# V-Sekai/godot-whisper

Hardware: AMD Instinct MI355X
Metric: realtime-factor (audio-sec/wall-sec), base.en 30 s chunk, PCM->tokens (higher is better)
Workload: dtype f16; 1 GPU; base.en, single 30 s chunk per step per GPU (1x MI355X), greedy decode, host params (max_tokens=16, single_segment, token_timestamps), whisper_full with host PCM (H2D inside the timed region); weights=synthetic seed 1234 (f16 ggml, base.en shape)

## Files before the change

### godot-whisper_amd/csrc/api.cpp

```cpp

#include <algorithm>
#include "wmi.h"
#include "kernels.h"

#include <chrono>
#include <cmath>
#include <cstdarg>
#include <cstring>
#include <mutex>
#include <exception>
#include <fstream>

namespace wmi {

namespace {
void default_log(ggml_log_level, const char * text, void *) { fputs(text, stderr); fflush(stderr); }
ggml_log_callback g_log_cb = default_log;
void * g_log_ud = nullptr;
std::recursive_mutex g_log_mu;
}

void log_msg(ggml_log_level lvl, const char * fmt, ...) {
    va_list ap, ap2;
    va_start(ap, fmt);
// ... 312 lines not shown
        ctx->dsp_scratch = nullptr; ctx->dsp_scratch_bytes = 0;
        if (!HIP_OK(hipMalloc((void **) &ctx->dsp_scratch, bytes))) return nullptr;
        ctx->dsp_scratch_bytes = bytes;
    }
    return ctx->dsp_scratch;
}

int wmi_downmix_stereo(struct whisper_context * ctx, const float * frames, int n_frames, int on_device, float * mono_out) {
    if (!ctx || !ctx->state || ctx->host_only || !frames || !mono_out || n_frames < 0) return -1;
    CtxScope lk(ctx);
    if (!HIP_OK(hipSetDevice(ctx->device))) return -2;
    hipStream_t s = ctx->state->dev.stream;
    if (n_frames == 0) return 0;
    if (on_device) { k::downmix_stereo(frames, n_frames, mono_out, s); return HIP_OK(hipStreamSynchronize(s)) ? 0 : -3; }
    float * d_in = dsp_scratch(ctx, (size_t) n_frames * 12), * d_out = d_in ? d_in + (size_t) n_frames * 2 : nullptr;
    bool ok = d_in && HIP_OK(hipMemcpyAsync(d_in, frames, (size_t) n_frames * 8, hipMemcpyHostToDevice, s));
    if (ok) k::downmix_stereo(d_in, n_frames, d_out, s);
    ok = ok && HIP_OK(hipMemcpyAsync(mono_out, d_out, (size_t) n_frames * 4, hipMemcpyDeviceToHost, s)) && HIP_OK(hipStreamSynchronize(s));
    return ok ? 0 : -3;
}

int wmi_resample(struct whisper_context * ctx, const float * src, int n_frames, int src_rate, int dst_rate, int converter, int on_device,
                 float * dst, int dst_capacity) {
    if (!ctx || !ctx->state || ctx->host_only || !src || !dst || n_frames < 0 || src_rate <= 0 || dst_rate <= 0 || dst_capacity < 0 ||
        converter < 0 || converter > 4) return -1;
    CtxScope lk(ctx);
    if (!HIP_OK(hipSetDevice(ctx->device))) return -2;
    hipStream_t s = ctx->state->dev.stream;
    if (src_rate == dst_rate) {
        if (n_frames > dst_capacity) return -4;
        const bool ok = n_frames == 0 || (HIP_OK(hipMemcpyAsync(dst, src, (size_t) n_frames * 4, on_device ? hipMemcpyDeviceToDevice : hipMemcpyHostToHost, s)) &&
                                          HIP_OK(hipStreamSynchronize(s)));
        return ok ? n_frames : -3;
    }
    const double ratio = (double) (uint32_t) dst_rate / (double) (uint32_t) src_rate;
    const long long out_frames = (int) ((uint32_t) n_frames * ratio);
    if (out_frames > dst_capacity) return -4;
    try {
    const k::ResamplePlan pl = k::resample_plan(n_frames, out_frames, ratio, converter);
    if (pl.error == -31) {
        WMI_ERR("wmi_resample: SRC_LINEAR cannot upsample a single frame, 0 frames\n");
        return 0;
    }
    if (pl.error) {
        WMI_ERR("wmi_resample: converter error %d (src_simple would report it through src_strerror)\n", -pl.error);
        return pl.error == -10 ? -10 : 0;
    }
    if (pl.n_out == 0) return 0;
    const float * d_tab = nullptr;
    bool ok = true;
    if (converter <= 2) {
        float *& d_sinc = ctx->d_sinc[converter];
        if (!d_sinc) {
            const float * coeffs; int count, inc;
            (void) k::sinc_table(converter, &coeffs, &count, &inc);
            ok = HIP_OK(hipMalloc((void **) &d_sinc, (size_t) count * 4)) && HIP_OK(hipMemcpyAsync(d_sinc, coeffs, (size_t) count * 4, hipMemcpyHostToDevice, s));
            if (!ok) { if (d_sinc) { (void) hipFree(d_sinc); d_sinc = nullptr; } return -3; }
        }
        d_tab = d_sinc;
    }
    float * d_in = nullptr, * d_out = nullptr; int * d_pos = nullptr; double * d_frac = nullptr;
    const float * in = src; float * out = dst;
    if (!on_device) {
        d_in = dsp_scratch(ctx, ((size_t) std::max(n_frames, 1) + (size_t) pl.n_out) * 4);
        d_out = d_in ? d_in + std::max(n_frames, 1) : nullptr;
        ok = d_in && HIP_OK(hipMemcpyAsync(d_in, src, (size_t) n_frames * 4, hipMemcpyHostToDevice, s));
        in = d_in; out = d_out;
    }
    if (ok && pl.need_table) {
        const int * hp; const double * hf;
        k::resample_table(pl, &hp, &hf);
        ok = HIP_OK(hipMalloc((void **) &d_pos, (size_t) pl.n_out * 4)) && HIP_OK(hipMalloc((void **) &d_frac, (size_t) pl.n_out * 8)) &&
             HIP_OK(hipMemcpyAsync(d_pos, hp, (size_t) pl.n_out * 4, hipMemcpyHostToDevice, s)) &&
             HIP_OK(hipMemcpyAsync(d_frac, hf, (size_t) pl.n_out * 8, hipMemcpyHostToDevice, s));
    }
    if (ok) k::resample_launch(pl, in, n_frames, out, d_tab, d_pos, d_frac, s);
    if (ok && !on_device) ok = HIP_OK(hipMemcpyAsync(dst, d_out, (size_t) pl.n_out * 4, hipMemcpyDeviceToHost, s));
    ok = ok && HIP_OK(hipStreamSynchronize(s));
    (void) hipFree(d_pos); (void) hipFree(d_frac);
    return ok ? (int) pl.n_out : -3;
    } catch (...) { WMI_ERR("wmi_resample: out of memory\n"); return -3; }
}

int wmi_selftest_ts_refine(struct whisper_context * ctx, const float * envelope, int n, const int * s0s1, int n_tok, float * sums, float * thold, int * walks) {
    if (!ctx || !envelope || n <= 0 || !s0s1 || n_tok <= 0 || n_tok > 4096 || !sums || !thold || !walks) return -1;
    CtxScope lk(ctx);
    if (!compute_ready(*ctx, __func__)) return -2;
    try {
        (void) hipSetDevice(ctx->device);
        const size_t nb = (size_t) n / 256 + 2;
        std::vector<float> ext(2 * nb, 0.0f);
        for (size_t b = 0; b * 256 < (size_t) n; ++b) {
            float lo = INFINITY, hi = -INFINITY;
            for (size_t i = b * 256; i < std::min<size_t>((b + 1) * 256, (size_t) n); ++i) { lo = std::min(lo, envelope[i]); hi = std::max(hi, envelope[i]); }
            ext[b] = lo; ext[nb + b] = hi;
        }
        std::vector<k::TsTok> in(n_tok);
        for (int t = 0; t < n_tok; ++t) {
            const int s0 = s0s1[2 * t], s1 = s0s1[2 * t + 1];
            if (s0 < 0 || s0 >= n || s1 < 0 || s1 >= n) return -1;
            in[t] = k::TsTok{ s0, s1, std::max(s0 - 2000, 0), std::min(s1 + 2000, n), nullptr, 0, 0 };
        }
        float * d_en = nullptr, * d_ext = nullptr; k::TsTok * d_in = nullptr; k::TsOut * d_out = nullptr;
        hipStream_t s = ctx->state->dev.stream;
        bool ok = HIP_OK(hipMalloc((void **) &d_en, (size_t) n * 4)) && HIP_OK(hipMalloc((void **) &d_ext, 2 * nb * 4)) &&
                  HIP_OK(hipMalloc((void **) &d_in, (size_t) n_tok * sizeof(k::TsTok))) && HIP_OK(hipMalloc((void **) &d_out, (size_t) n_tok * sizeof(k::TsOut)));
        std::vector<k::TsOut> out(n_tok);
        if (ok) {
            ok = HIP_OK(hipMemcpyAsync(d_en, envelope, (size_t) n * 4, hipMemcpyHostToDevice, s)) &&
                 HIP_OK(hipMemcpyAsync(d_ext, ext.data(), 2 * nb * 4, hipMemcpyHostToDevice, s)) &&
                 HIP_OK(hipMemcpyAsync(d_in, in.data(), (size_t) n_tok * sizeof(k::TsTok), hipMemcpyHostToDevice, s));
            if (ok) k::ts_refine(d_en, d_ext, d_ext + nb, n, d_in, d_out, n_tok, s);
            ok = ok && HIP_OK(hipMemcpyAsync(out.data(), d_out, (size_t) n_tok * sizeof(k::TsOut), hipMemcpyDeviceToHost, s)) && HIP_OK(hipStreamSynchronize(s));
        }
        if (d_en) (void) hipFree(d_en); if (d_ext) (void) hipFree(d_ext); if (d_in) (void) hipFree(d_in); if (d_out) (void) hipFree(d_out);
        if (!ok) return -3;
        for (int t = 0; t < n_tok; ++t) {
            sums[t] = out[t].sum; thold[t] = out[t].thold;
            int * w = walks + 6 * t;
            w[0] = out[t].e0; w[1] = out[t].e1; w[2] = out[t].w_down_above_s0; w[3] = out[t].w_up_below_s0; w[4] = out[t].w_up_above_s1; w[5] = out[t].w_down_below_s1;
        }
        return 0;
    } catch (const std::exception & e) {
        WMI_ERR("%s: %s\n", __func__, e.what());
        return -9;
    }
}

int wmi_selftest_greedy_step(struct whisper_context * ctx, whisper_token token, int pos, float * logits, whisper_token_data * out, int * forms) {
    if (!ctx || ctx->host_only || !out) return -1;
    CtxScope lk(ctx);
    if (!compute_ready(*ctx, __func__)) return -2;
    (void) hipSetDevice(ctx->device);
    BusyScope busy(ctx->device);
    const Vocab & v = ctx->model.vocab;
    if (pos < 0 || pos >= ctx->model.hp.n_text_ctx || token < 0 || token >= v.n_vocab) return -1;
    if (!upload_static_ban(*ctx, whisper_full_default_params(WHISPER_SAMPLING_GREEDY))) return -3;
    StepFilter f{};
    f.ban_blank = false; f.last_ts = false; f.penult_ts = false; f.ts_floor_end = v.beg; f.ts_initial_start = v.n_vocab;
    unsigned fm = 0;
    if (!decode_greedy_step(*ctx, token, pos, f, *out, &fm)) return -4;
    if (logits) {
        DeviceState & d = ctx->state->dev;
        if (!HIP_OK(hipMemcpyAsync(logits, d.logits, (size_t) ctx->model.hp.n_vocab * 4, hipMemcpyDeviceToHost, d.stream)) ||
            !HIP_OK(hipStreamSynchronize(d.stream))) return -5;
    }
    if (forms) *forms = (int) fm;
    return 0;
}

int wmi_selftest_filters(struct whisper_context * ctx, struct whisper_full_params params, int mode, int n_rows, const float * logits,
                         const whisper_token * hist, const int * n_hist, const int * has_ts, const int * seek_delta, float temperature,
                         const void * W, const float * x, int K, float * logits_out, const double * u, int k, int tid_default,
                         whisper_token_data * out) {
    if (!ctx || !ctx->state || !out || !n_hist || !has_ts || !seek_delta || mode < 0 || mode > 2) return -1;
    if (mode == 0 && (n_rows < 1 || n_rows > 16 || !logits)) return -1;
    if (mode == 1 && (n_rows != 1 || !W || !x || !logits_out || K <= 0)) return -1;
    if (mode == 2 && (n_rows < 1 || n_rows > 8 || k < 1 || k > 8 || !logits || !u)) return -1;
    if (mode != 2) k = 1;
    for (int r = 0; r < n_rows; ++r) if (n_hist[r] < 0 || (n_hist[r] > 0 && !hist)) return -1;
    const Vocab & v = ctx->model.vocab; const HParams & hp = ctx->model.hp;
    const int NV = v.n_vocab;
    k::GemvArgs g{};
    if (mode == 1) {
        static const float one = 1.0f; static k::FsPartial none;
        g.ln_g = &one; g.fs_part = &none;
        g.eps = hp.eps; g.n = 1; g.K = K; g.N = NV; g.epi = k::EPI_LOGITS; g.ldc = NV; g.ldr = K; g.ldaux = K; g.ldaux2 = K; g.S = K;
        if (k::gemv_fused_parts(g) <= 0) return -4;
    }
    CtxScope lk(ctx);
    if (!compute_ready(*ctx, __func__)) return -2;
    struct DevBufs {
        std::vector<void *> p;
        ~DevBufs() { for (void * q : p) (void) hipFree(q); }
        void * get(size_t bytes) { void * q = nullptr; if (!HIP_OK(hipMalloc(&q, bytes))) return nullptr; p.push_back(q); return q; }
    } bufs;
    try {
// ... 1323 lines not shown
```

### godot-whisper_amd/csrc/batch.cpp

```cpp

#include "wmi.h"
#include "kernels.h"

#include <algorithm>
#include <cmath>
#include <cstdlib>
#include <cstring>
#include <thread>
#include <mutex>

namespace wmi {

namespace {

constexpr int MAX_LANES = 16;

template <typename T> bool dalloc(T *& p, size_t n_elems) {
    p = nullptr;
    return HIP_OK(hipMalloc((void **) &p, std::max<size_t>(n_elems, 1) * sizeof(T)));
}
template <typename T> void dfree(T *& p) { if (p) (void) hipFree(p); p = nullptr; }

struct StateSwap {
    StateInstall inst;
    StateSwap(whisper_context & c, State * lane) : inst(c.state, lane) {}
};

State * new_lane_state(whisper_context & ctx) {
    State * st = new State();
    st->dev.stream = ctx.state->dev.stream;
    if (!dalloc(st->dev.mel_max, 4)) { delete st; return nullptr; }
    if (!HIP_OK(hipStreamCreateWithFlags(&st->dev.mel_stream, hipStreamNonBlocking)) ||
        !HIP_OK(hipEventCreateWithFlags(&st->dev.mel_ev, hipEventDisableTiming))) { delete st; return nullptr; }
    for (auto & dec : st->decoders) dec.rng = std::mt19937(0);
    return st;
}

void free_lane_state(State * st) {
    DeviceState & d = st->dev;
    if (d.copy_stream) { (void) hipStreamSynchronize(d.copy_stream); (void) hipStreamDestroy(d.copy_stream); }
    if (d.energy_ev) (void) hipEventDestroy(d.energy_ev);
    if (d.mel_stream) { (void) hipStreamSynchronize(d.mel_stream); (void) hipStreamDestroy(d.mel_stream); }
    if (d.mel_ev) (void) hipEventDestroy(d.mel_ev);
    dfree(d.pcm); dfree(d.mel); dfree(d.mel_max); dfree(d.energy);
    if (d.energy_host) (void) hipHostFree(d.energy_host);
    if (d.ts_host) (void) hipHostFree(d.ts_host);
    delete st;
}

bool ensure_batch(whisper_context & ctx, int B) {
    if (!ctx.batch) ctx.batch = new BatchWork();
    BatchWork & w = *ctx.batch;
    if (w.B >= B) return true;
    hipStream_t s = ctx.state->dev.stream;
    (void) hipStreamSynchronize(s);
    dfree(w.mel_t); dfree(w.conv1); dfree(w.x); dfree(w.xn); dfree(w.q); dfree(w.k); dfree(w.att); dfree(w.vt); dfree(w.h);
    dfree(w.enc_out_h); dfree(w.kvc_k); dfree(w.kvc_v); dfree(w.self_k); dfree(w.self_v); dfree(w.dx); dfree(w.dq); dfree(w.datt); dfree(w.dh);
    dfree(w.logits); dfree(w.xattn); dfree(w.aq); dfree(w.ads); dfree(w.aq16); dfree(w.wq16); dfree(w.att32); dfree(w.datt32);
    for (auto & rg : w.rows_graph) {
        if (rg.exec) (void) hipGraphExecDestroy(rg.exec);
        if (rg.graph) (void) hipGraphDestroy(rg.graph);
        rg = BatchWork::RowsGraph{};
    }
    w.chain_valid = false;
    if (w.front_hand) (void) hipFree(w.front_hand);
    if (w.step_dev) (void) hipFree(w.step_dev);
    if (w.sample_dev) (void) hipFree(w.sample_dev);
    if (w.filter_scratch) (void) hipFree(w.filter_scratch);
    if (w.step_host) (void) hipHostFree(w.step_host);
    if (w.sample_host) (void) hipHostFree(w.sample_host);
    if (w.lang_host) (void) hipHostFree(w.lang_host);
    w.step_dev = w.sample_dev = w.filter_scratch = w.step_host = w.sample_host = nullptr; w.lang_host = nullptr;

    const HParams & hp = ctx.model.hp;
    const size_t S = hp.n_audio_state, T = hp.n_audio_ctx, Lt = hp.n_text_layer, H = hp.n_audio_head, n_ctx = hp.n_text_ctx;
    w.Tpad = (int) ((T + 63) / 64 * 64);
    w.mel_rows = 2 * T + 8;
    const size_t nb = (size_t) B;
    const size_t TP = (T + 15) & ~(size_t) 15;
    bool ok = dalloc(w.mel_t, nb * w.mel_rows * hp.n_mels + 1024) && dalloc(w.conv1, nb * (2 * T + 8) * S + 4 * S)
           && dalloc(w.x, nb * TP * S) && dalloc(w.xn, nb * TP * S) && dalloc(w.q, nb * TP * S) && dalloc(w.k, nb * TP * S)
           && dalloc(w.att, nb * TP * S) && dalloc(w.vt, nb * S * w.Tpad) && dalloc(w.h, nb * TP * 4 * S) && dalloc(w.enc_out_h, nb * TP * S)
           && dalloc(w.kvc_k, Lt * nb * TP * S) && dalloc(w.kvc_v, Lt * nb * TP * S)
           && dalloc(w.self_k, nb * Lt * n_ctx * S) && dalloc(w.self_v, nb * Lt * n_ctx * S)
           && dalloc(w.dx, nb * S) && dalloc(w.dq, nb * S) && dalloc(w.datt, nb * S) && dalloc(w.dh, nb * 4 * S) && dalloc(w.logits, nb * hp.n_vocab)
           && dalloc(w.xattn, k::attn_cross_scratch_floats(B, (int) H, (int) T));
    if (ctx.model.quantised) {
        w.aq_rows = (int) (nb * TP);
        ok = ok && dalloc(w.aq, nb * TP * 4 * S) && dalloc(w.ads, 2 * nb * TP * (4 * S / 32)) && dalloc(w.att32, nb * TP * S) && dalloc(w.datt32, nb * S);
        w.wq16_elems = 8 * S * S;
        ok = ok && dalloc(w.aq16, nb * TP * 4 * S) && dalloc(w.wq16, w.wq16_elems);
    }
    if (ok && !ctx.model.quantised && S <= 1024) {
        const size_t bytes = nb * 16 * S + 64 + nb * (size_t) k::XBACK_ROW_GRANULES * 8;
        if (HIP_OK(hipMalloc(&w.front_hand, bytes))) k::fill_zero(w.front_hand, bytes, ctx.state->dev.stream); else w.front_hand = nullptr;
    }
    ok = ok && HIP_OK(hipMalloc(&w.step_dev, nb * sizeof(k::DecStep))) && HIP_OK(hipMalloc(&w.sample_dev, nb * sizeof(k::SampleOut)))
            && HIP_OK(hipMalloc(&w.filter_scratch, k::filter_scratch_bytes(B)))
            && HIP_OK(hipHostMalloc(&w.step_host, nb * sizeof(k::DecStep), hipHostMallocDefault))
            && HIP_OK(hipHostMalloc(&w.sample_host, nb * sizeof(k::SampleOut), hipHostMallocDefault))
            && HIP_OK(hipHostMalloc((void **) &w.lang_host, nb * k::LANG_HEAD_N * sizeof(float), hipHostMallocDefault));
    if (!ok) { WMI_ERR("%s: device allocation failed (B = %d)\n", __func__, B); w.B = 0; return false; }
    memset(w.sample_host, 0, nb * sizeof(k::SampleOut));
    w.step_seq = 0;
    k::fill_zero(w.vt, nb * S * w.Tpad * sizeof(__half), s);
    k::fill_zero(w.xn, nb * TP * S * sizeof(__half), s);
    k::fill_zero(w.x, nb * TP * S * sizeof(float), s);
    k::fill_zero(w.att, nb * TP * S * sizeof(__half), s);
    if (ctx.model.quantised) k::fill_zero(w.att32, nb * TP * S * sizeof(float), s);
    k::fill_zero(w.conv1, (nb * (2 * T + 8) * S + 4 * S) * sizeof(__half), s);
    k::fill_zero(w.mel_t, (nb * w.mel_rows * hp.n_mels + 1024) * sizeof(__half), s);
    k::fill_zero(w.self_k, nb * Lt * n_ctx * S * sizeof(__half), s);
    k::fill_zero(w.self_v, nb * Lt * n_ctx * S * sizeof(__half), s);
    k::fill_zero(w.kvc_k, Lt * nb * TP * S * sizeof(__half), s);
    k::fill_zero(w.kvc_v, Lt * nb * TP * S * sizeof(__half), s);
    HIP_TRY(hipStreamSynchronize(s));
    if (w.lanes.empty()) w.lanes.push_back(ctx.state);
    while ((int) w.lanes.size() < B) {
        State * st = new_lane_state(ctx);
        if (!st) return false;
        w.lanes.push_back(st);
    }
    w.B = B;
    return true;
}

}

bool encode_rows(whisper_context & ctx, const std::vector<int> & rows, const std::vector<int> & seek, int audio_ctx, const int * row_ctx) {
// ... 653 lines not shown
            std::vector<char> all_det(n_chunks, 0); std::vector<float> all_probs((size_t) n_chunks * k::LANG_HEAD_N, 0.0f);
            for (int g = 0; g < G; ++g) c0[g + 1] = c0[g] + n_chunks / G + (g < n_chunks % G ? 1 : 0);
            int64_t tm[4] = {0, 0, 0, 0}; int steps = 0, chained = 0;
            std::mutex merge_mu;
            auto work = [&](int g) {
                try {
                    whisper_context & wc = g == 0 ? ctx : *ctx.batch->replicas[g - 1];
                    (void) hipSetDevice(ctx.device);
                    if (g > 0 && wc.batch) wc.batch->groups_wanted = 1;
                    wc.no_speech_mode = nsm; wc.token_dtw_mode = ctx.token_dtw_mode; wc.dtw_pairs = ctx.dtw_pairs; wc.grammar_device_mode = ctx.grammar_device_mode;
                    t_in_group = true;
                    struct Off { ~Off() { t_in_group = false; } } off;
                    const int cnt = c0[g + 1] - c0[g];
                    struct Ordered { bool was; Ordered() : was(t_ordered) { t_ordered = true; } ~Ordered() { t_ordered = was; } } ordered;
                    const int rc = full_batch(wc, params, pcm + c0[g], n_samples + c0[g], cnt, on_device, audio_ctx ? audio_ctx + c0[g] : nullptr);
                    rets[g] = rc;
                    if (rc != 0 || !wc.batch) return;
                    std::lock_guard<std::mutex> lk(merge_mu);
                    for (int i = 0; i < cnt; ++i) {
                        all[c0[g] + i] = std::move(wc.batch->results[i]); all_win[c0[g] + i] = std::move(wc.batch->windows[i]); all_redo[c0[g] + i] = wc.batch->redo[i];
                        all_lang[c0[g] + i] = wc.batch->lang_id[i]; all_det[c0[g] + i] = wc.batch->lang_detected[i];
                        std::copy_n(wc.batch->lang_probs.begin() + (size_t) i * k::LANG_HEAD_N, k::LANG_HEAD_N, all_probs.begin() + (size_t) (c0[g] + i) * k::LANG_HEAD_N);
                    }
                    tm[0] = std::max(tm[0], wc.batch->t_mel_us); tm[1] = std::max(tm[1], wc.batch->t_encode_us);
                    tm[2] = std::max(tm[2], wc.batch->t_decode_us); tm[3] = std::max(tm[3], wc.batch->t_emit_us);
                    steps = std::max(steps, wc.batch->n_steps); chained = std::max(chained, wc.batch->n_chained);
                } catch (const std::exception & e) {
                    WMI_ERR("wmi_full_batch: lock-step group %d: %s\n", g, e.what());
                    rets[g] = -10;
                } catch (...) { rets[g] = -10; }
            };
            {
                std::vector<std::thread> th;
                struct Joiner { std::vector<std::thread> & t; ~Joiner() { for (auto & x : t) if (x.joinable()) x.join(); } } joiner{th};
                for (int g = 1; g < G; ++g) th.emplace_back(work, g);
                work(0);
            }
            for (int g = 0; g < G; ++g) if (rets[g] != 0) return rets[g];
            BatchWork & bw = *ctx.batch;
            bw.results = std::move(all); bw.windows = std::move(all_win); bw.redo = std::move(all_redo);
            bw.lang_id = std::move(all_lang); bw.lang_detected = std::move(all_det); bw.lang_probs = std::move(all_probs);
            bw.t_mel_us = tm[0]; bw.t_encode_us = tm[1]; bw.t_decode_us = tm[2]; bw.t_emit_us = tm[3]; bw.n_steps = steps; bw.n_chained = chained;
            bw.groups_last = G;
            return 0;
        }
    }
    ctx.batch->groups_last = 1;
    const int max_lanes = k::rows_valu_enabled() ? 8 : MAX_LANES;
    if (!ensure_batch(ctx, std::min(n_chunks, max_lanes))) return -2;
    BatchWork & b = *ctx.batch;
    if (!upload_static_ban(ctx, params)) return -7;
    struct EnvelopeGuard { BatchWork & b; ~EnvelopeGuard() { for (State * l : b.lanes) (void) signal_energy_wait(*l); } } envelope_guard{b};

    const bool has_fallback = params.temperature_inc > 0.0f && params.temperature + params.temperature_inc < 1.0f + 1e-6f;
    std::vector<int32_t> prompt_user;
    if (!params.prompt_tokens && params.initial_prompt) {
        prompt_user = tokenize(v, params.initial_prompt);
        if (prompt_user.size() > 1024) {
            WMI_ERR("%s: too many resulting tokens: %d (max %d)\n", "whisper_tokenize", (int) prompt_user.size(), 1024);
            prompt_user.clear();
        }
    } else if (params.prompt_tokens && params.prompt_n_tokens > 0) {
        prompt_user.assign(params.prompt_tokens, params.prompt_tokens + params.prompt_n_tokens);
    }
    auto prompt_init_of = [&](int lid) {
        std::vector<int32_t> pi = { v.sot };
        if (v.is_multilingual()) {
            pi.push_back(v.sot + 1 + lid);
            pi.push_back(params.translate ? v.translate : v.transcribe);
        }
        if (params.no_timestamps) pi.push_back(v.not_);
        return pi;
    };
    const int lid_known = lang_known && v.is_multilingual() ? lang_id(params.language) : 0;
    int space_id = -1;
    { auto sp = v.token_to_id.find(" "); if (sp != v.token_to_id.end()) space_id = sp->second; }
    const int n_max = hp.n_text_ctx / 2 - 4;

    const int group = std::min(b.B, max_lanes);
    for (int g0 = 0; g0 < n_chunks; g0 += group) {
        const int ng = std::min(group, n_chunks - g0);
        if (!lang_known) for (int r = 0; r < ng; ++r) if (n_samples[g0 + r] <= 0) { WMI_ERR("%s: failed to auto-detect language (chunk %d is empty)\n", __func__, g0 + r); return -3; }
        std::vector<Row> rows(ng);
        static const bool ts_device = !(getenv("WMI_TS_DEVICE") && atoi(getenv("WMI_TS_DEVICE")) == 0);
        static const bool mel_per_chunk = getenv("WMI_MEL_PER_CHUNK") != nullptr;
        const bool env_batched = params.token_timestamps && ts_device;
        const bool mel_batched = !mel_per_chunk && ng >= 2 && (env_batched || !params.token_timestamps);
        if (mel_batched) {
            const int64_t tm0 = time_us();
            std::vector<State *> sts(ng);
            for (int r = 0; r < ng; ++r) sts[r] = b.lanes[r];
            if (!pcm_to_mel_batch(ctx, sts, pcm + g0, n_samples + g0, on_device, env_batched)) { WMI_ERR("%s: failed to compute log mel spectrogram\n", __func__); return -2; }
            b.t_mel_us += time_us() - tm0;
        }
        for (int r = 0; r < ng; ++r) {
            Row & row = rows[r]; row.chunk = g0 + r; row.lane = r;
            State & ls = *b.lanes[r];
            StateSwap sw(ctx, &ls);
            ls.result_all.clear();
            ls.windows.clear();
            ls.ts_failed = false;
            ls.prompt_past = prompt_user;
            ls.exp_n_audio_ctx = actx(row.chunk);
            if (v.is_multilingual() && lang_known) ls.lang_id = lid_known;
            ls.lang_probs.clear();
            const int64_t tm0 = time_us();
            if (n_samples[row.chunk] > 0 && !mel_batched) {
                if (!pcm_to_mel(ctx, pcm[row.chunk], n_samples[row.chunk], on_device, false)) { WMI_ERR("%s: failed to compute log mel spectrogram\n", __func__); return -2; }
            }
            if (params.token_timestamps) {
                ls.t_beg = 0; ls.t_last = 0; ls.tid_last = 0;
                if (!mel_batched && n_samples[row.chunk] > 0 && !signal_energy_device(ctx, 32, false, ts_device ? 3 : 0)) { WMI_ERR("%s: failed to compute the signal envelope\n", __func__); return -2; }
            }
            b.t_mel_us += time_us() - tm0;
        }
        {
            const int64_t tm0 = time_us();
            for (int r = 0; r < ng; ++r) {
                DeviceState & ld = b.lanes[r]->dev;
                if (mel_batched || !ld.mel_stream || n_samples[g0 + r] <= 0) continue;
                if (!HIP_OK(hipEventRecord(ld.mel_ev, ld.mel_stream)) || !HIP_OK(hipStreamWaitEvent(primary->dev.stream, ld.mel_ev, 0))) return -2;
            }
            if (!HIP_OK(hipStreamSynchronize(primary->dev.stream))) return -2;
            b.t_mel_us += time_us() - tm0;
        }
        for (int r = 0; r < ng; ++r) {
            Row & row = rows[r]; State & ls = *b.lanes[r];
            row.seek_start = params.offset_ms / 10;
            row.seek_end = params.duration_ms == 0 ? ls.mel.n_len_org : row.seek_start + params.duration_ms / 10;
            row.seek = row.seek_start;
            row.live = row.seek_end >= row.seek_start + 100;
        }

        bool enc_at_0 = false;
        if (!lang_known) {
            std::vector<int> lanes(ng), seeks(ng, 0);
            for (int r = 0; r < ng; ++r) {
                lanes[r] = r;
                if (b.lanes[r]->mel.n_len_org <= 0) { WMI_ERR("%s: failed to auto-detect language\n", __func__); return -3; }
            }
            if (!encode_rows(ctx, lanes, seeks, 0)) { WMI_ERR("%s: failed to encode\n", __func__); return -3; }
            const int64_t td0 = time_us();
            k::DecStep * hs = (k::DecStep *) b.step_host;
            ++b.step_seq;
            for (int r = 0; r < ng; ++r) {
                memset(&hs[r], 0, sizeof(k::DecStep));
                hs[r].token = v.sot; hs[r].pos = 0; hs[r].n_kv = 1; hs[r].kv_head = 0; hs[r].seq = b.step_seq;
                hs[r].space_id = space_id; hs[r].eot = v.eot; hs[r].beg = v.beg; hs[r].n_vocab = v.n_vocab;
                hs[r].ts_floor_end = v.beg; hs[r].ts_initial_start = v.n_vocab;
            }
            b.chain_valid = false;
            enqueue_rows_step(ctx, ng, false, 0, b.lang_host);
            if (!HIP_OK(hipStreamSynchronize(primary->dev.stream)) || !HIP_OK(hipGetLastError())) { WMI_ERR("%s: failed to decode\n", __func__); return -3; }
            b.chain_valid = false;
            for (int r = 0; r < ng; ++r) {
                State & ls = *b.lanes[r];
                ls.lang_probs.assign(k::LANG_HEAD_N, 0.0f);
                ls.lang_id = lang_probs_from_logits(b.lang_host + (size_t) r * k::LANG_HEAD_N, ls.lang_probs.data());
            }
            b.t_decode_us += time_us() - td0; b.n_steps++;
            enc_at_0 = true;
        }
        for (int r = 0; r < ng; ++r) {
            const State & ls = *b.lanes[r];
            keep_lang(g0 + r, ls);
            rows[r].prompt_init = prompt_init_of(ls.lang_id);
        }
// ... 179 lines not shown
```

### godot-whisper_amd/csrc/device.cpp

```cpp

#include "wmi.h"
#include <atomic>
#include <thread>
#include <map>
#include <mutex>
#include "kernels.h"

#include <algorithm>
#include <cmath>
#include <cstdlib>
#include <cstring>

namespace wmi {

namespace {

template <typename T> bool dalloc(T *& p, size_t n_elems) {
    p = nullptr;
    return HIP_OK(hipMalloc((void **) &p, std::max<size_t>(n_elems, 1) * sizeof(T)));
}
template <typename T> void dfree(T *& p) { if (p) (void) hipFree(p); p = nullptr; }

}

// ... 61 lines not shown
        static const int spares = getenv("WMI_SPARE_QUEUES") ? atoi(getenv("WMI_SPARE_QUEUES"))
                                : getenv("WMI_BATCH_REPLICAS") ? std::max(0, std::min(15, atoi(getenv("WMI_BATCH_REPLICAS")))) : 3;
        for (int i = 0; i < spares; ++i) { hipStream_t sp = own_queue_stream_get(ctx.device); if (sp) ctx.spare_streams.push_back(sp); }
    }

    const size_t S = hp.n_audio_state, T = hp.n_audio_ctx, Lt = hp.n_text_layer, H = hp.n_audio_head;
    const size_t n_self = 3 * (size_t) hp.n_text_ctx;
    st->kv_self.size = (uint32_t) n_self; st->kv_self.cells.assign(n_self, KVCell());
    bool ok = true;
    ok = ok && dalloc(st->kv_self.k, Lt * n_self * S) && dalloc(st->kv_self.v, Lt * n_self * S);
    ok = ok && dalloc(d.kvc_k, Lt * T * S) && dalloc(d.kvc_v, Lt * T * S);
    d.Tpad = (int) ((T + 63) / 64 * 64);
    const size_t mel_rows = 2 * T + 8;
    ok = ok && dalloc(d.mel_t, mel_rows * hp.n_mels + 1024) && dalloc(d.conv1, (2 * T + 4) * S)
            && dalloc(d.x, T * S) && dalloc(d.embd_conv, T * S) && dalloc(d.xn, T * S)
            && dalloc(d.q, T * S) && dalloc(d.k, T * S) && dalloc(d.vt, S * d.Tpad) && dalloc(d.att, T * S)
            && dalloc(d.h, T * 4 * S) && dalloc(d.rowmax, H * T) && dalloc(d.enc_out, T * S) && dalloc(d.enc_out_h, T * S)
            && dalloc(d.mel_max, 4);
    const size_t n = hp.n_text_ctx;
    if (ctx.model.quantised) {
        const size_t rows = std::max<size_t>(T, n);
        d.aq_rows = (int) rows;
        ok = ok && dalloc(d.aq, rows * 4 * S) && dalloc(d.ads, 2 * rows * (4 * S / 32)) && dalloc(d.att32, T * S) && dalloc(d.datt32, n * S);
        d.wq16_elems = 8 * S * S;
        ok = ok && dalloc(d.aq16, rows * 4 * S) && dalloc(d.wq16, d.wq16_elems);
    }
    d.logits_rows_cap = 8;
    ok = ok && dalloc(d.d_tokens, 3 * n + n * n_self);
    if (ok) { d.d_pos = d.d_tokens + n; d.d_rows = d.d_pos + n; d.d_mask = (float *) (d.d_rows + n); }
    ok = ok
            && dalloc(d.dx, n * S) && dalloc(d.dxn, n * S) && dalloc(d.dq, n * S) && dalloc(d.datt, n * S)
            && dalloc(d.dh, n * 4 * S) && dalloc(d.logits, (size_t) d.logits_rows_cap * hp.n_vocab)
            && dalloc(d.xattn, k::attn_cross_scratch_floats((int) n, (int) H, (int) T));
    d.pinned_bytes = std::max<size_t>((size_t) d.logits_rows_cap * hp.n_vocab * 4, n * n_self * 4 + 3 * n * 4 + 4096);
    ok = ok && HIP_OK(hipHostMalloc(&d.pinned, d.pinned_bytes, hipHostMallocDefault));
    {
        unsigned char * hand = nullptr;
        const size_t hand_bytes = (size_t) 32 * S + 64 + 40960 + (size_t) 8 * S;
        ok = ok && dalloc(hand, hand_bytes);
        if (ok) { d.mlp_hand = hand; d.mlp_arrive = (unsigned long long *) (hand + (size_t) 16 * S); k::fill_zero(hand, hand_bytes, d.stream); }
    }
    if (!ok) { WMI_ERR("%s: device allocation failed\n", __func__); return false; }
    k::fill_zero(d.vt, S * d.Tpad * sizeof(__half), d.stream);
    k::fill_zero(d.conv1, (2 * T + 4) * S * sizeof(__half), d.stream);
    k::fill_zero(d.mel_t, (mel_rows * hp.n_mels + 1024) * sizeof(__half), d.stream);
    k::fill_zero(st->kv_self.k, Lt * n_self * S * sizeof(__half), d.stream);
    k::fill_zero(st->kv_self.v, Lt * n_self * S * sizeof(__half), d.stream);
    k::fill_zero(d.kvc_k, Lt * T * S * sizeof(__half), d.stream);
    k::fill_zero(d.kvc_v, Lt * T * S * sizeof(__half), d.stream);
    HIP_TRY(hipStreamSynchronize(d.stream));

    st->batch.token.resize(n); st->batch.pos.resize(n); st->batch.seq_id.resize(n); st->batch.logits.resize(n);
    st->logits.reserve((size_t) hp.n_vocab * 8);
    for (auto & dec : st->decoders) dec.rng = std::mt19937(0);
    WMI_INFO("%s: kv self size = %.2f MB, kv cross size = %.2f MB\n", __func__,
             2.0 * Lt * n_self * S * 2 / 1e6, 2.0 * Lt * T * S * 2 / 1e6);
    return true;
}

State * create_state(whisper_context & ctx) {
    State * st = new State();
    if (init_state_into(ctx, st, true, nullptr)) return st;
    destroy_state(st);
    return nullptr;
}

void free_state(whisper_context & ctx) {
    destroy_state(ctx.state);
    ctx.state = nullptr;
}

void destroy_state(State * st) {
    if (!st) return;
    (void) hipSetDevice(st->device);
    DeviceState & d = st->dev;
    if (d.stream) (void) hipStreamSynchronize(d.stream);
    dfree(st->kv_self.k); dfree(st->kv_self.v); dfree(d.kvc_k); dfree(d.kvc_v);
    if (d.copy_stream) { (void) hipStreamSynchronize(d.copy_stream); (void) hipStreamDestroy(d.copy_stream); }
    if (d.energy_ev) (void) hipEventDestroy(d.energy_ev);
    for (hipEvent_t & e : d.ph_ev) { if (e) (void) hipEventDestroy(e); e = nullptr; }
    if (d.mel_ev) { (void) hipEventDestroy(d.mel_ev); d.mel_ev = nullptr; }
    dfree(d.energy); if (d.energy_host) (void) hipHostFree(d.energy_host);
    if (d.ts_host) (void) hipHostFree(d.ts_host);
    dfree(d.pcm); dfree(d.mel); dfree(d.mel_max); dfree(d.mel_t); dfree(d.conv1); dfree(d.x); dfree(d.embd_conv);
    dfree(d.xn); dfree(d.q); dfree(d.k); dfree(d.vt); dfree(d.att); dfree(d.h); dfree(d.rowmax); dfree(d.enc_out);
    dfree(d.enc_out_h); dfree(d.d_tokens); d.d_pos = nullptr; d.d_mask = nullptr; d.d_rows = nullptr; dfree(d.dx); dfree(d.dxn);
    dfree(d.dq); dfree(d.datt); dfree(d.dh); dfree(d.logits); dfree(d.xattn); dfree(d.ban_dev);
    if (d.mlp_hand) { (void) hipFree(d.mlp_hand); d.mlp_hand = nullptr; d.mlp_arrive = nullptr; }
    dfree(d.aq); dfree(d.ads); dfree(d.aq16); dfree(d.wq16); dfree(d.att32); dfree(d.datt32);
    for (auto & sg : d.step_graphs) { if (sg.exec) (void) hipGraphExecDestroy(sg.exec); if (sg.graph) (void) hipGraphDestroy(sg.graph); sg = DeviceState::StepGraph{}; }
    if (d.step_dev) (void) hipFree(d.step_dev);
    if (d.sample_dev) (void) hipFree(d.sample_dev);
    if (d.filter_scratch) (void) hipFree(d.filter_scratch);
    if (d.draw_scratch) (void) hipFree(d.draw_scratch);
    if (d.draw_host) (void) hipHostFree(d.draw_host);
    dfree(d.gram.vbytes); dfree(d.gram.voff); dfree(d.gram.rules); dfree(d.gram.states); dfree(d.gram.reject);
    if (d.gram.scratch) (void) hipFree(d.gram.scratch);
    if (d.gram.host) (void) hipHostFree(d.gram.host);
    if (d.step_host) (void) hipHostFree(d.step_host);
    if (d.sample_host) (void) hipHostFree(d.sample_host);
    if (d.nsp_scratch) (void) hipFree(d.nsp_scratch);
    dfree(d.nsp_logits);
    if (d.nsp_host) (void) hipHostFree(d.nsp_host);
    for (void * q : { (void *) d.dtw.w, (void *) d.dtw.mu, (void *) d.dtw.sigma, (void *) d.dtw.A, (void *) d.dtw.cost, (void *) d.dtw.trace, (void *) d.dtw.q })
        if (q) (void) hipFree(q);
    if (d.dtw_host) (void) hipHostFree(d.dtw_host);
    if (d.score_scratch) (void) hipFree(d.score_scratch);
    dfree(d.score_items); dfree(d.score_lp);
    if (d.score_host) (void) hipHostFree(d.score_host);
    if (d.draft_part) (void) hipFree(d.draft_part);
    if (d.draft_dev) (void) hipFree(d.draft_dev);
    if (d.draft_host) (void) hipHostFree(d.draft_host);
    if (d.pinned) (void) hipHostFree(d.pinned);
    if (d.stream && d.stream_own_queue) own_queue_stream_put(st->device, d.stream);
    else if (d.stream) (void) hipStreamDestroy(d.stream);
    delete st;
}

static bool ensure_mel_capacity(DeviceState & d, size_t n_pad, size_t n_mel_elems) {
    if (n_pad > d.pcm_cap) { dfree(d.pcm); if (!dalloc(d.pcm, n_pad + 1024)) return false; d.pcm_cap = n_pad + 1024; }
    if (n_mel_elems > d.mel_cap) { dfree(d.mel); if (!dalloc(d.mel, n_mel_elems)) return false; d.mel_cap = n_mel_elems; }
    return true;
}

static bool phase_events(DeviceState & d) {
    for (hipEvent_t & e : d.ph_ev) if (!e && !HIP_OK(hipEventCreate(&e))) return false;
    return true;
}
int64_t phase_settle(State & st, bool wait) {
    DeviceState & d = st.dev;
    if (!d.ph_mel && !d.ph_enc) return 0;
    if (wait) (void) hipStreamSynchronize(d.stream);
    float ms = 0.0f; double gpu_us = 0.0;
    if (d.ph_mel) { if (hipEventSynchronize(d.ph_ev[1]) == hipSuccess && hipEventElapsedTime(&ms, d.ph_ev[0], d.ph_ev[1]) == hipSuccess) { st.t_mel_us += (int64_t) (ms * 1e3); gpu_us += ms * 1e3; } d.ph_mel = false; }
    if (d.ph_enc) { if (hipEventSynchronize(d.ph_ev[3]) == hipSuccess && hipEventElapsedTime(&ms, d.ph_ev[2], d.ph_ev[3]) == hipSuccess) { st.t_encode_us += (int64_t) (ms * 1e3); gpu_us += ms * 1e3; } d.ph_enc = false; }
    return d.ph_host0 + (int64_t) gpu_us;
}

bool pcm_to_mel(whisper_context & ctx, const float * samples, int n_samples, bool samples_on_device, bool sync, bool defer) {
    if (!compute_ready(ctx, __func__)) return false;
    State & st = *ctx.state; DeviceState & d = st.dev;
    const int64_t t0 = time_us();
    const int n_mel = ctx.model.n_filt_mel;
    hipStream_t ms = d.mel_stream ? d.mel_stream : d.stream;
    const int64_t n_pad = (int64_t) n_samples + 480000 + 400;
    const int n_len = (int) ((n_pad - 400) / 160);
    const int n_len_org = 1 + (n_samples + 200 - 400) / 160;
    const int n_valid = n_samples + 200;
    const int n_fft_frames = std::min(n_valid / 160 + 1, n_len);
    if (!ensure_mel_capacity(d, (size_t) n_pad + (size_t) n_samples, (size_t) n_mel * n_len)) return false;
    defer = defer && ms == d.stream && phase_events(d);
    if (defer) { (void) phase_settle(st, true); HIP_TRY(hipEventRecord(d.ph_ev[0], ms)); }
    const float * src = samples;
    if (!samples_on_device) {
        float * stage = d.pcm + n_pad;
        if (WavJob * job = d.pcm_job) {
            d.pcm_job = nullptr;
            if (!wav_job_run(ctx, *job, stage, ms)) return false;
        } else HIP_TRY(hipMemcpyAsync(stage, samples, (size_t) n_samples * 4, hipMemcpyHostToDevice, ms));
        src = stage;
    }
    d.last_pcm = src; d.last_pcm_n = n_samples;
    k::mel_pad(src, n_samples, d.pcm, (int) n_pad, ms, (int *) d.mel_max);
    k::mel_frames(d.pcm, n_valid, n_fft_frames, n_len, n_mel, ctx.w.mel_filters, ctx.w.mel_ranges, ctx.w.mel_taps, d.mel, (int *) d.mel_max, ms);
    k::mel_normalize(d.mel, n_mel * n_len, (const int *) d.mel_max, ms);
    st.mel.n_len = n_len; st.mel.n_len_org = n_len_org; st.mel.n_mel = n_mel;
// ... 24 lines not shown
    if (envelopes && !ensure_copy_stream(pd)) return false;
    for (size_t r = 0; r < states.size(); ++r) {
        const int n = n_samples[r];
        if (n <= 0) continue;
        if (nb >= 16) return false;
        State & st = *states[r]; DeviceState & d = st.dev;
        const int64_t n_pad = (int64_t) n + 480000 + 400;
        const int n_len = (int) ((n_pad - 400) / 160);
        if (!ensure_mel_capacity(d, (size_t) n_pad + (size_t) n, (size_t) n_mel * n_len)) return false;
        const float * src = pcm[r];
        if (!samples_on_device) {
            float * stage = d.pcm + n_pad;
            HIP_TRY(hipMemcpyAsync(stage, pcm[r], (size_t) n * 4, hipMemcpyHostToDevice, s));
            src = stage;
        }
        d.last_pcm = src; d.last_pcm_n = n;
        st.mel.n_len = n_len; st.mel.n_len_org = 1 + (n + 200 - 400) / 160; st.mel.n_mel = n_mel;
        mb.pcm[nb] = src; mb.pad[nb] = d.pcm; mb.mel[nb] = d.mel; mb.gmax[nb] = (int *) d.mel_max; mb.n[nb] = n;
        if (envelopes) {
            if (d.energy_pending && envelope_stream(d)) { HIP_TRY(hipStreamSynchronize(envelope_stream(d))); d.energy_pending = false; }
            const size_t nblk = (size_t) n / 256 + 2;
            if ((size_t) n > d.energy_cap) {
                st.energy = nullptr; st.energy_n = 0; st.energy_bmin = st.energy_bmax = nullptr;
                if (d.energy_host) (void) hipHostFree(d.energy_host);
                d.energy_host = nullptr; d.energy_cap = 0;
                if (!HIP_OK(hipHostMalloc((void **) &d.energy_host, ((size_t) n + 2 * ((size_t) n / 256 + 2)) * 4, hipHostMallocDefault))) return false;
                d.energy_cap = (size_t) n;
            }
            const size_t need = d.energy_cap + 2 * nblk;
            if (d.energy_dev_cap < need) { dfree(d.energy); d.energy_dev_cap = 0; if (!dalloc(d.energy, need)) return false; d.energy_dev_cap = need; }
            mb.energy[nb] = d.energy; mb.bmin[nb] = d.energy + d.energy_cap; mb.bmax[nb] = d.energy + d.energy_cap + nblk;
        }
        in.push_back(&st); ++nb;
    }
    if (nb == 0) return true;
    if (envelopes) {
        if (!pd.mel_ev) HIP_TRY(hipEventCreateWithFlags(&pd.mel_ev, hipEventDisableTiming));
        HIP_TRY(hipEventRecord(pd.energy_ev, s));
        HIP_TRY(hipStreamWaitEvent(pd.copy_stream, pd.energy_ev, 0));
        k::signal_energy_batch(mb, nb, 32, pd.copy_stream);
        HIP_TRY(hipEventRecord(pd.mel_ev, pd.copy_stream));
        for (State * st : in) {
            DeviceState & d = st->dev;
            d.energy_device_only = true; d.energy_pending = true; d.energy_wait_stream = pd.copy_stream;
        }
    }
    k::mel_batch(mb, nb, n_mel, ctx.w.mel_filters, ctx.w.mel_ranges, ctx.w.mel_taps, s);
    if (envelopes) HIP_TRY(hipStreamWaitEvent(s, pd.mel_ev, 0));
    ctx.state->t_mel_us += time_us() - t0;
    return hipGetLastError() == hipSuccess;
}

bool signal_energy_device(whisper_context & ctx, int hw, bool sync, int via_dma) {
    State & st = *ctx.state; DeviceState & d = st.dev;
    const int n = d.last_pcm_n;
    if (!d.last_pcm || n <= 0) return false;
    if (!ensure_copy_stream(d)) return false;
    if (d.energy_pending) { HIP_TRY(hipStreamSynchronize(envelope_stream(d))); d.energy_pending = false; }
    d.energy_wait_stream = nullptr;
    d.energy_device_only = false;
    if ((size_t) n > d.energy_cap) {
        st.energy = nullptr; st.energy_n = 0; st.energy_bmin = st.energy_bmax = nullptr;
        if (d.energy_host) (void) hipHostFree(d.energy_host);
        d.energy_host = nullptr; d.energy_cap = 0;
        if (!HIP_OK(hipHostMalloc((void **) &d.energy_host, ((size_t) n + 2 * ((size_t) n / 256 + 2)) * 4, hipHostMallocDefault))) return false;
        d.energy_cap = (size_t) n;
    }
    HIP_TRY(hipEventRecord(d.energy_ev, d.mel_stream ? d.mel_stream : d.stream));
    HIP_TRY(hipStreamWaitEvent(d.copy_stream, d.energy_ev, 0));
    {
        const size_t nb = (size_t) n / 256 + 2;
        const size_t need = d.energy_cap + 2 * nb;
        if (via_dma && d.energy_dev_cap < need) { dfree(d.energy); d.energy_dev_cap = 0; if (dalloc(d.energy, need)) d.energy_dev_cap = need; else via_dma = 0; }
        if (via_dma == 3) {
            k::signal_energy(d.last_pcm, n, hw, d.energy, d.energy + d.energy_cap, d.energy + d.energy_cap + nb, d.copy_stream);
            d.energy_device_only = true;
        } else
        k::signal_energy(d.last_pcm, n, hw, d.energy_host, d.energy_host + d.energy_cap, d.energy_host + d.energy_cap + nb, d.copy_stream);
    }
    d.energy_pending = true;
    return sync ? signal_energy_wait(st) : true;
}

bool ts_refine_device(State & st, const k::TsTok * in, int n, k::TsOut * out) {
    DeviceState & d = st.dev;
    constexpr int CAP = 448;
    if (n <= 0) return true;
    hipStream_t es = envelope_stream(d);
    if (n > CAP || !d.energy || !es) return false;
    if (!d.ts_host && !HIP_OK(hipHostMalloc(&d.ts_host, CAP * (sizeof(k::TsTok) + sizeof(k::TsOut)), hipHostMallocDefault))) return false;
    k::TsTok * hin = (k::TsTok *) d.ts_host; k::TsOut * hout = (k::TsOut *) (hin + CAP);
    memcpy(hin, in, (size_t) n * sizeof(k::TsTok));
    const size_t nb = (size_t) d.last_pcm_n / 256 + 2;
    k::ts_refine(d.energy, d.energy + d.energy_cap, d.energy + d.energy_cap + nb, d.last_pcm_n, hin, hout, n, es);
    HIP_TRY(hipStreamSynchronize(es));
    memcpy(out, hout, (size_t) n * sizeof(k::TsOut));
    return true;
}

bool signal_energy_wait(State & st) {
    DeviceState & d = st.dev;
    if (!d.energy_pending) return true;
    if (d.energy_device_only) {
        HIP_TRY(hipStreamSynchronize(envelope_stream(d)));
        st.energy = nullptr; st.energy_bmin = st.energy_bmax = nullptr; st.energy_n = d.last_pcm_n; st.energy_on_device = true;
        d.energy_pending = false;
        return true;
    }
    st.energy_on_device = false;
    HIP_TRY(hipStreamSynchronize(d.copy_stream));
    st.energy = d.energy_host; st.energy_n = d.last_pcm_n;
    st.energy_bmin = d.energy_host + d.energy_cap; st.energy_bmax = st.energy_bmin + ((size_t) d.last_pcm_n / 256 + 2);
    d.energy_pending = false;
    return true;
}

bool set_mel(whisper_context & ctx, const float * data, int n_len, int n_mel) {
    if (!compute_ready(ctx, __func__)) return false;
    State & st = *ctx.state; DeviceState & d = st.dev;
    if (!ensure_mel_capacity(d, 0, (size_t) n_len * n_mel)) return false;
    HIP_TRY(hipMemcpyAsync(d.mel, data, (size_t) n_len * n_mel * 4, hipMemcpyHostToDevice, d.stream));
    HIP_TRY(hipStreamSynchronize(d.stream));
    st.mel.n_len = n_len; st.mel.n_len_org = n_len; st.mel.n_mel = n_mel;
    return true;
}

bool encode(whisper_context & ctx, int mel_offset, bool defer) {
    if (!compute_ready(ctx, __func__)) return false;
    State & st = *ctx.state; DeviceState & d = st.dev; const Weights & w = ctx.w; const HParams & hp = ctx.model.hp;
    const int64_t t0 = time_us();
    d.chain_valid = false;
    defer = defer && !ctx.model.quantised && phase_events(d);
    if (defer) {
        if (d.ph_enc) (void) phase_settle(st, true);
        HIP_TRY(hipEventRecord(d.ph_ev[2], d.stream));
        if (!d.ph_mel) d.ph_host0 = t0;
    }
    const int T = st.exp_n_audio_ctx > 0 ? st.exp_n_audio_ctx : hp.n_audio_ctx;
    const int S = hp.n_audio_state, H = hp.n_audio_head, La = hp.n_audio_layer, Lt = hp.n_text_layer, nm = hp.n_mels;
    hipStream_t s = d.stream;
    if (st.mel.n_mel != nm || d.mel == nullptr) { WMI_ERR("%s: no mel spectrogram (n_mel %d, expected %d)\n", __func__, st.mel.n_mel, nm); return false; }

    const int rows_mel = 2 * T + 6;
    k::mel_slice(d.mel, st.mel.n_len, nm, mel_offset, 2 * T, d.mel_t, nm, rows_mel, s);
    {
        k::GemmArgs a{};
        a.A = d.mel_t; a.lda = nm; a.W = w.conv1_w; a.ldw = w.conv1_k; a.M = 2 * T; a.N = S; a.K = w.conv1_k;
        a.bias = w.conv1_b; a.C = d.conv1 + S; a.ldc = S;
        k::gemm(k::EPI_F16_BIAS_GELU, a, s);
    }
    if (d.conv1_max_T > T) k::fill_zero(d.conv1 + (size_t) (2 * T + 1) * S, (size_t) S * sizeof(__half), s);
    d.conv1_max_T = std::max(d.conv1_max_T, T);
    {
        k::GemmArgs a{};
        a.A = d.conv1; a.lda = 2 * S; a.W = w.conv2_w; a.ldw = w.conv2_k; a.M = T; a.N = S; a.K = w.conv2_k;
        a.bias = w.conv2_b; a.C = d.x; a.ldc = S; a.resid = w.e_pe; a.ldr = S; a.aux = d.embd_conv; a.ldaux = S;
        k::gemm(k::EPI_CONV2, a, s);
    }
    const float kq_scale = 1.0f / sqrtf((float) S / H);
    if (ctx.model.quantised) { if (!encode_layers_q(ctx, T)) return false; }
    else {
    for (int il = 0; il < La; ++il) {
        const EncLayerW & l = w.enc[il];
        k::layernorm(d.x, T, S, l.ln1_g, l.ln1_b, hp.eps, d.xn, nullptr, s);
        {
            k::GemmArgs a{};
            a.A = d.xn; a.lda = S; a.W = l.w_qkv; a.ldw = S; a.M = T; a.N = 3 * S; a.K = S; a.bias = l.b_qkv;
            a.C = d.q; a.ldc = S; a.aux = d.k; a.ldaux = S; a.aux2 = d.vt; a.ldaux2 = d.Tpad; a.S = S;
            k::gemm(k::EPI_QKV_ENC, a, s);
        }
        k::attn_encoder(d.q, d.k, d.vt, T, d.Tpad, S, H, kq_scale, d.att, s);
        {
            k::GemmArgs a{};
            a.A = d.att; a.lda = S; a.W = l.w_o; a.ldw = S; a.M = T; a.N = S; a.K = S; a.bias = l.b_o;
            a.C = d.x; a.ldc = S; a.resid = d.x; a.ldr = S;
            k::gemm(k::EPI_F32_BIAS_RESID, a, s);
        }
        k::layernorm(d.x, T, S, l.ln2_g, l.ln2_b, hp.eps, d.xn, nullptr, s);
        {
            k::GemmArgs a{};
// ... 1002 lines not shown
```

### godot-whisper_amd/csrc/full.cpp

```cpp

#include "wmi.h"

#include <algorithm>
#include <immintrin.h>
#include <climits>
#include <cmath>
#include <cstdint>
#include <cstdlib>
#include <cstring>
#include <thread>

namespace wmi {

namespace {

constexpr int MAX_DECODERS = 8;

struct BeamCandidate { int decoder_idx; int seek_delta; bool has_ts; Sequence sequence; Grammar grammar; };

const char * tok_str(whisper_context & ctx, int32_t id) { return ctx.model.vocab.id_to_token.at(id).c_str(); }

void emit_segment(whisper_context & ctx, State & st, const whisper_full_params & params, int64_t t0, int64_t t1, const std::string & text,
                  const std::vector<whisper_token_data> & toks, int i0, int i1_excl, bool speaker_turn_next) {
    const int64_t tt0 = params.speed_up ? 2 * t0 : t0, tt1 = params.speed_up ? 2 * t1 : t1;
    if (params.print_realtime) {
        if (params.print_timestamps) {
            auto stamp = [](int64_t t, char (&buf)[32]) {
                const int64_t ms = t * 10;
                snprintf(buf, sizeof(buf), "%02d:%02d:%02d.%03d", (int) (ms / 3600000), (int) ((ms / 60000) % 60), (int) ((ms / 1000) % 60), (int) (ms % 1000));
            };
            char b0[32], b1[32];
            stamp(tt0, b0); stamp(tt1, b1);
            printf("[%s --> %s]  %s\n", b0, b1, text.c_str());
        }
        else { printf("%s", text.c_str()); fflush(stdout); }
    }
    Segment seg{tt0, tt1, text, {}, speaker_turn_next};
    seg.tokens.assign(toks.begin() + i0, toks.begin() + i1_excl);
    seg.i_tok0 = i0;
    st.result_all.push_back(std::move(seg));
    int n_new = 1;
    if (params.token_timestamps) {
        (void) signal_energy_wait(st);
        token_level_timestamps(ctx, st, (int) st.result_all.size() - 1, params.thold_pt, params.thold_ptsum);
        if (params.max_len > 0) n_new = wrap_segment(ctx, st, params.max_len, params.split_on_word);
    }
    if (params.new_segment_callback)
        params.new_segment_callback(&ctx, (whisper_state *) &st, n_new, params.new_segment_callback_user_data);
}

}

bool align_window(whisper_context & ctx, State & st, int seek, int seek_end, const std::vector<int32_t> & prompt_init, const Decoder & best, int32_t seg0);

void decoder_advance(const whisper_context & ctx, const whisper_full_params & params, Decoder & d, int i, int seek, int seek_end, int n_max) {
    const Vocab & v = ctx.model.vocab;
    int & result_len = d.sequence.result_len;
    const whisper_token_data & tok = d.sequence.tokens.back();
    if (tok.id > v.beg) {
        const int sd_new = 2 * (tok.id - v.beg);
        if (d.has_ts && d.seek_delta > sd_new && result_len < i) { d.failed = true; return; }
        d.seek_delta = sd_new; result_len = i + 1; d.has_ts = true;
    }
    grammar_accept_token(ctx, d.grammar, tok.id);
    if (tok.id == v.eot || (params.max_tokens > 0 && i >= params.max_tokens) ||
        (d.has_ts && seek + d.seek_delta + 100 >= seek_end)) {
        if (result_len == 0) {
            if (seek + d.seek_delta + 100 >= seek_end) result_len = i + 1;
            else { d.failed = true; return; }
        }
        if (params.single_segment) { result_len = i + 1; d.seek_delta = 100 * WHISPER_CHUNK_SIZE; }
        d.completed = true;
        return;
    }
    if (ctx.model.n_loaded == 0) { d.seek_delta = 100 * WHISPER_CHUNK_SIZE; d.completed = true; return; }
    if (i == n_max - 1 && (result_len == 0 || d.seek_delta < 100 * WHISPER_CHUNK_SIZE / 2)) { d.failed = true; return; }
}

DraftPlan draft_plan(const whisper_context & ctx, const whisper_full_params & params, int P, const int32_t * draft, int n_offered, int seek, int seek_end) {
    const Vocab & v = ctx.model.vocab; const HParams & hp = ctx.model.hp;
    const int n_max = hp.n_text_ctx / 2 - 4;
    DraftPlan pl;
    int n = std::min(n_offered, n_max - 1);
    if (params.max_tokens > 0) n = std::min(n, params.max_tokens + 1);
    n = std::min(n, hp.n_text_ctx - P - 1);
    pl.n = std::max(0, n);
    Decoder dd;
    dd.seek_delta = 100 * WHISPER_CHUNK_SIZE;
    pl.filters.reserve((size_t) pl.n + 1);
    for (int j = 0; j <= pl.n; ++j) {
        pl.filters.push_back(make_step_filter(v, hp, params, dd));
        if (j == pl.n) break;
        dd.sequence.tokens.push_back(whisper_token_data{ draft[j], 0, 0.f, 0.f, 0.f, 0.f, -1, -1, 0.f });
        if (!dd.completed && !dd.failed) decoder_advance(ctx, params, dd, j, seek, seek_end, n_max);
    }
    return pl;
}

int full(whisper_context & ctx, whisper_full_params params, const float * samples, const float * d_samples, int n_samples) {
    BusyScope busy(ctx.device);
    State & st = *ctx.state;
    const Vocab & v = ctx.model.vocab;
    const HParams & hp = ctx.model.hp;
    st.result_all.clear();
    speaker_invalidate(ctx);
    st.ts_failed = false;
    st.lang_probs.clear();
    std::vector<int32_t> draft_tokens; draft_tokens.swap(st.draft);
    float * const draft_logits_out = st.draft_logits_out; const int draft_logits_cap = st.draft_logits_cap;
    st.draft_logits_out = nullptr; st.draft_logits_cap = 0;
    st.draft_status = { (int32_t) draft_tokens.size(), 0, 0, 0, draft_tokens.empty() ? 1 : 2 };
    bool first_window = true;
    const int nsm = ctx.no_speech_mode;
    st.windows.clear();
    const bool dtw = ctx.token_dtw_mode != 0 && ctx.model.n_loaded > 0;
    if (dtw) st.dtw_pairs_call = ctx.dtw_pairs.empty() ? dtw_default_pairs(hp) : ctx.dtw_pairs;
    st.dtw_last = State::DtwDims{}; st.dtw_jumps.clear();
    st.gram_steps_dev = 0; st.gram_rows_host = 0;
    const bool gram_mode = ctx.grammar_device_mode == 1 && params.grammar_rules && params.n_grammar_rules > 0 && ctx.model.n_loaded > 0;
    GrammarFlat gram_flat;
    if (gram_mode) gram_flat = grammar_flatten(grammar_init(params.grammar_rules, params.n_grammar_rules, params.i_start_rule));
    struct EnvelopeGuard { State & st; ~EnvelopeGuard() { (void) signal_energy_wait(st); } } envelope_guard{st};
    static const bool defer_phases = getenv("WMI_PHASE_SYNC") == nullptr;
    struct PhaseGuard { State & st; ~PhaseGuard() { (void) phase_settle(st, true); } } phase_guard{st};

    if (n_samples > 0) {
        if (params.speed_up) { WMI_ERR("%s: failed to compute log mel spectrogram\n", __func__); return -1; }
        const bool ok_mel = d_samples ? pcm_to_mel(ctx, d_samples, n_samples, true, true, defer_phases) : pcm_to_mel(ctx, samples, n_samples, false, true, defer_phases);
        if (!ok_mel) { WMI_ERR("%s: failed to compute log mel spectrogram\n", __func__); return -2; }
    }

    int enc_at_0 = 0;
    if (params.language == nullptr || strlen(params.language) == 0 || strcmp(params.language, "auto") == 0 || params.detect_language) {
        std::vector<float> probs(lang_max_id() + 1, 0.0f);
        const bool head = k::lang_head_usable(hp.n_text_state);
        const int lid = head ? lang_detect_head(ctx, 0, probs.data(), defer_phases) : lang_auto_detect(ctx, 0, probs.data());
        if (lid < 0) { WMI_ERR("%s: failed to auto-detect language\n", __func__); return -3; }
        enc_at_0 = st.enc_n_ctx;
        st.lang_probs = probs;
        st.lang_id = lid;
        params.language = lang_str(lid);
        WMI_INFO("%s: auto-detected language: %s (p = %f)\n", __func__, params.language, probs[lid]);
        if (params.detect_language) return 0;
    }

    if (params.token_timestamps) {
        st.t_beg = 0; st.t_last = 0; st.tid_last = 0;
        if (n_samples > 0 && !signal_energy_device(ctx, 32, false)) { WMI_ERR("%s: failed to compute the signal envelope\n", __func__); return -2; }
    }

    const int seek_start = params.offset_ms / 10;
    const int seek_end = params.duration_ms == 0 ? st.mel.n_len_org : seek_start + params.duration_ms / 10;
    if (seek_end < seek_start + (params.speed_up ? 50 : 100)) return 0;

    std::vector<float> temperatures;
    if (params.temperature_inc > 0.0f) for (float t = params.temperature; t < 1.0f + 1e-6f; t += params.temperature_inc) temperatures.push_back(t);
    else temperatures.push_back(params.temperature);

    int n_decoders = 1;
    if (params.strategy == WHISPER_SAMPLING_GREEDY) n_decoders = params.greedy.best_of;
    else if (params.strategy == WHISPER_SAMPLING_BEAM_SEARCH) n_decoders = std::max(params.greedy.best_of, params.beam_search.beam_size);
    n_decoders = std::max(1, n_decoders);
    if (n_decoders > MAX_DECODERS) { WMI_ERR("%s: too many decoders requested (%d), max = %d\n", __func__, n_decoders, MAX_DECODERS); return -4; }
    for (int j = 1; j < n_decoders; ++j) {
        Decoder & d = st.decoders[j];
        d.probs.resize(v.n_vocab); d.logits.resize(v.n_vocab); d.logprobs.resize(v.n_vocab);
        d.rng = std::mt19937(0);
    }

    auto & prompt_past = st.prompt_past;
    if (params.no_context) prompt_past.clear();
    std::vector<int32_t> prompt_tokens_own;
    if (!params.prompt_tokens && params.initial_prompt) {
        prompt_tokens_own = tokenize(v, params.initial_prompt);
        if (prompt_tokens_own.size() > 1024) {
            WMI_ERR("%s: too many resulting tokens: %d (max %d)\n", "whisper_tokenize", (int) prompt_tokens_own.size(), 1024);
            prompt_tokens_own.clear();
        }
        params.prompt_tokens = prompt_tokens_own.data();
        params.prompt_n_tokens = (int) prompt_tokens_own.size();
    }
    if (params.prompt_tokens && params.prompt_n_tokens > 0) {
        for (int i = 0; i < params.prompt_n_tokens; ++i) prompt_past.push_back(params.prompt_tokens[i]);
        std::rotate(prompt_past.begin(), prompt_past.end() - params.prompt_n_tokens, prompt_past.end());
    }

    if (params.audio_ctx > hp.n_audio_ctx) {
        WMI_ERR("%s: audio_ctx is larger than the maximum allowed (%d > %d)\n", __func__, params.audio_ctx, hp.n_audio_ctx);
        return -5;
    }
    st.exp_n_audio_ctx = params.audio_ctx;

    std::vector<int32_t> prompt_init = { v.sot };
    if (v.is_multilingual()) {
        const int lid = lang_id(params.language);
        st.lang_id = lid;
        prompt_init.push_back(v.sot + 1 + lid);
        prompt_init.push_back(params.translate ? v.translate : v.transcribe);
    }
    if (hp.n_text_layer == 2 && !params.no_timestamps) {
        WMI_WARN("%s: using distilled model - forcing no_timestamps\n", __func__);
        params.no_timestamps = true;
    }
    if (params.no_timestamps) prompt_init.push_back(v.not_);

    int seek = seek_start;
    std::vector<int32_t> prompt;
    prompt.reserve(hp.n_text_ctx);
    std::vector<std::vector<BeamCandidate>> bc_per_dec(n_decoders);
    std::vector<BeamCandidate> beam_candidates;
    const bool beam = params.strategy == WHISPER_SAMPLING_BEAM_SEARCH;

    while (true) {
        if (params.progress_callback)
            params.progress_callback(&ctx, (whisper_state *) ctx.state.get(), (100 * (seek - seek_start)) / (seek_end - seek_start),
                                     params.progress_callback_user_data);
        if (seek + 100 >= seek_end) break;
        if (params.encoder_begin_callback &&
            !params.encoder_begin_callback(&ctx, (whisper_state *) ctx.state.get(), params.encoder_begin_callback_user_data)) {
            WMI_ERR("%s: encoder_begin_callback returned false - aborting\n", __func__);
            break;
        }
        const bool encoded = enc_at_0 > 0 && seek == 0 && enc_at_0 == (st.exp_n_audio_ctx > 0 ? st.exp_n_audio_ctx : hp.n_audio_ctx);
        enc_at_0 = 0;
        if ((!encoded && !encode(ctx, seek, defer_phases)) || (params.abort_callback && params.abort_callback(params.abort_callback_user_data))) {
            WMI_ERR("%s: failed to encode\n", __func__);
            return -6;
        }
        if (seek > seek_start && seek + 500 >= seek_end) prompt_past.clear();

        int best_decoder_id = 0;
// ... 398 lines not shown
            for (int k = 0; k < B; k += 8) {
                const __m256 t = _mm256_mul_ps(_mm256_loadu_ps(p + i + k), vs);
                const __m256i q = _mm256_cvtps_epi32(t);
                const __m256 d = _mm256_and_ps(_mm256_sub_ps(t, _mm256_cvtepi32_ps(q)), absmask);
                bad = _mm256_or_ps(bad, _mm256_cmp_ps(d, half, _CMP_EQ_OQ));
                bad = _mm256_or_ps(bad, _mm256_cmp_ps(t, big, _CMP_NLT_UQ));
                bad = _mm256_or_ps(bad, _mm256_cmp_ps(t, _mm256_setzero_ps(), _CMP_LT_OQ));
                isum = _mm256_add_epi32(isum, q);
            }
            if (_mm256_movemask_ps(bad) == 0) {
                __m128i s4 = _mm_add_epi32(_mm256_castsi256_si128(isum), _mm256_extracti128_si256(isum, 1));
                s4 = _mm_add_epi32(s4, _mm_shuffle_epi32(s4, 0x4E)); s4 = _mm_add_epi32(s4, _mm_shuffle_epi32(s4, 0xB1));
                const uint64_t total = (uint64_t) units + (uint32_t) _mm_cvtsi128_si32(s4);
                if (total < 0x1000000u) {
                    const uint32_t nb = ((uint32_t) (E + 127) << 23) | ((uint32_t) total & 0x7FFFFFu);
                    memcpy(&acc, &nb, 4);
                    i += B;
                    continue;
                }
            }
        }
        const int e = std::min(n, i + B);
        for (; i < e; ++i) acc += p[i];
    }
    return acc;
}

void ts_collect(whisper_context & ctx, State & st, std::vector<k::TsTok> & in, std::vector<TsRef> & ref) {
    const Vocab & v = ctx.model.vocab;
    const int n_samples = st.energy_n;
    const int hw = WHISPER_SAMPLE_RATE / 8;
    for (int si : st.ts_pending) {
        auto & tokens = st.result_all[si].tokens;
        for (int j = 0; j < (int) tokens.size(); ++j) {
            if (tokens[j].id >= v.eot) continue;
            const int s0 = ts_to_sample(tokens[j].t0, n_samples), s1 = ts_to_sample(tokens[j].t1, n_samples);
            in.push_back(k::TsTok{ s0, s1, std::max(s0 - hw, 0), std::min(s1 + hw, n_samples), st.dev.energy, n_samples, (int32_t) st.dev.energy_cap });
            ref.push_back(TsRef{ &st, si, j });
        }
    }
    st.ts_pending.clear();
}

void ts_apply(const std::vector<k::TsTok> & in, const std::vector<TsRef> & ref, const std::vector<k::TsOut> & res) {
    for (size_t q = 0; q < ref.size(); ++q) {
        auto & tokens = ref[q].st->result_all[ref[q].seg].tokens;
        const int n = (int) tokens.size(), j = ref[q].j;
        const k::TsOut & r = res[q];
        int s0 = in[q].s0, s1 = in[q].s1;
        const int ns = in[q].a1 - in[q].a0;
        if (r.e0 && j > 0) {
            const int k2 = r.w_down_above_s0;
            tokens[j].t0 = sample_to_ts(k2);
            if (tokens[j].t0 < tokens[j - 1].t1) tokens[j].t0 = tokens[j - 1].t1; else s0 = k2;
        } else {
            const int k2 = r.w_up_below_s0;
            s0 = k2;
            tokens[j].t0 = sample_to_ts(k2);
        }
        if (r.e1) {
            const int k2 = r.w_up_above_s1;
            tokens[j].t1 = sample_to_ts(k2);
            if (j < ns - 1 && j + 1 < n && tokens[j].t1 > tokens[j + 1].t0) tokens[j].t1 = tokens[j + 1].t0; else s1 = k2;
        } else {
            const int k2 = s1 <= s0 ? s1 : std::max(s0, r.w_down_below_s1);
            s1 = k2;
            tokens[j].t1 = sample_to_ts(k2);
        }
        (void) s1;
    }
}

bool flush_token_timestamps(whisper_context & ctx, State & st) {
    if (st.ts_pending.empty() || st.ts_hold) return true;
    std::vector<State *> one{ &st };
    return flush_token_timestamps_of(ctx, one);
}
bool flush_token_timestamps_of(whisper_context & ctx, const std::vector<State *> & states) {
    std::vector<k::TsTok> in; std::vector<TsRef> ref;
    State * first = nullptr;
    std::vector<State *> involved;
    for (State * s : states) if (s && !s->ts_pending.empty()) { if (!first) first = s; involved.push_back(s); ts_collect(ctx, *s, in, ref); }
    if (!first || in.empty()) return true;
    std::vector<k::TsOut> res(in.size());
    for (size_t q0 = 0; q0 < in.size(); q0 += 448) {
        const int cnt = (int) std::min<size_t>(448, in.size() - q0);
        if (!ts_refine_device(*first, in.data() + q0, cnt, res.data() + q0)) {
            WMI_ERR("%s: timestamp refinement on the device failed\n", __func__);
            for (State * s : involved) s->ts_failed = true;
            return false;
        }
    }
    ts_apply(in, ref, res);
    return true;
}

void token_level_timestamps(whisper_context & ctx, State & st, int i_segment, float thold_pt, float thold_ptsum) {
    const Vocab & v = ctx.model.vocab;
    Segment & seg = st.result_all[i_segment];
    auto & tokens = seg.tokens;
    const int n_samples = st.energy_n;
    if (n_samples == 0) { WMI_ERR("%s: no signal data available\n", __func__); return; }
    const int64_t t0 = seg.t0, t1 = seg.t1;
    const int n = (int) tokens.size();
    if (n == 0) return;
    if (n == 1) { tokens[0].t0 = t0; tokens[0].t1 = t1; return; }

    for (int j = 0; j < n; ++j) {
        whisper_token_data & tok = tokens[j];
        if (j == 0) {
            if (tok.id == v.beg) {
                tokens[0].t0 = t0; tokens[0].t1 = t0; tokens[1].t0 = t0;
                st.t_beg = t0; st.t_last = t0; st.tid_last = v.beg;
            } else {
                tokens[0].t0 = st.t_last;
            }
        }
        const int64_t tt = st.t_beg + 2 * (tok.tid - v.beg);
        tok.vlen = voice_length(tok_str(ctx, tok.id));
        if (tok.pt > thold_pt && tok.ptsum > thold_ptsum && tok.tid > st.tid_last && tt <= t1) {
            if (j > 0) tokens[j - 1].t1 = tt;
            tok.t0 = tt;
            st.tid_last = tok.tid;
        }
    }
    tokens[n - 2].t1 = t1; tokens[n - 1].t0 = t1; tokens[n - 1].t1 = t1;
    st.t_last = t1;

    for (int p0 = 0, p1 = 0;;) {
        while (p1 < n && tokens[p1].t1 < 0) ++p1;
        if (p1 >= n) --p1;
        if (p1 > p0) {
            double psum = 0.0;
            for (int j = p0; j <= p1; ++j) psum += tokens[j].vlen;
            const double dt = (double) (tokens[p1].t1 - tokens[p0].t0);
            for (int j = p0 + 1; j <= p1; ++j) {
                const double ct = tokens[j - 1].t0 + dt * tokens[j - 1].vlen / psum;
                tokens[j - 1].t1 = (int64_t) ct;
                tokens[j].t0 = (int64_t) ct;
            }
        }
        ++p1; p0 = p1;
        if (p1 >= n) break;
    }
    for (int j = 0; j < n - 1; ++j) {
        if (tokens[j].t1 < 0) tokens[j + 1].t0 = tokens[j].t1;
        if (j > 0 && tokens[j - 1].t1 > tokens[j].t0) {
            tokens[j].t0 = tokens[j - 1].t1;
            tokens[j].t1 = std::max(tokens[j].t0, tokens[j].t1);
        }
    }

    const int hw = WHISPER_SAMPLE_RATE / 8;
    if (st.energy_on_device && st.ts_defer) { st.ts_pending.push_back(i_segment); return; }
    if (st.energy_on_device) {
        st.ts_pending.assign(1, i_segment);
        std::vector<State *> one{ &st };
        (void) flush_token_timestamps_of(ctx, one);
        return;
    }
    const float * en = st.energy;
    const float * bmin = st.energy_bmin, * bmax = st.energy_bmax;
    auto walk_down_while_above = [&](int k, float th) {
        while (k > 0 && en[k] > th) {
            if ((k & 255) == 255 && bmin && bmin[k >> 8] > th) {
                int b = k >> 8;
// ... 120 lines not shown
```

### godot-whisper_amd/csrc/k_mel.hip

```cpp

#include "kernels.h"
#include <type_traits>
#include "wave_ops.h"
#include <climits>
#include <cmath>
#include <mutex>

namespace wmi { namespace k {

namespace {

struct MelTables { float hann[400]; float sinv[400]; float cosv[400]; };
__constant__ MelTables c_mel;

std::atomic<uint64_t> g_tables_mask{0};

void upload_tables() {
    MelTables t;
    for (int i = 0; i < 400; ++i) {
        t.hann[i] = 0.5 * (1.0 - cosf((2.0 * M_PI * i) / 400));
        double theta = (2 * M_PI * i) / 400;
        t.sinv[i] = sinf(theta);
        t.cosv[i] = cosf(theta);
    }
// ... 361 lines not shown
    const size_t stride = (size_t) gridDim.x * blockDim.x;
    for (; i < n; i += stride) p[i] = 0u;
}

__global__ void k_set_int(int * p, int v) { *p = v; }

}

void mel_pad(const float * pcm, int n_samples, float * pcm_pad, int n_pad_total, hipStream_t st, int * gmax_reset) {
    hipLaunchKernelGGL(k_mel_pad, dim3((n_pad_total + 255) / 256), dim3(256), 0, st, pcm, n_samples, pcm_pad, n_pad_total, gmax_reset);
}

void mel_frames(const float * pcm_pad, int n_valid, int n_fft_frames, int n_len, int n_mel, const float * filters,
                const int32_t * ranges, const float * taps, float * mel, int * gmax, hipStream_t st) {
    {
        int dev = 0; (void) hipGetDevice(&dev);
        const uint64_t bit = 1ull << (dev & 63);
        if (!(g_tables_mask.load(std::memory_order_acquire) & bit)) { upload_tables(); g_tables_mask.fetch_or(bit, std::memory_order_release); }
    }
    if (n_fft_frames > 0)
        hipLaunchKernelGGL(k_mel_frames, dim3(n_fft_frames), dim3(MEL_NT), 0, st, pcm_pad, n_valid, n_fft_frames, n_len, n_mel,
                           filters, ranges, taps, mel, gmax);
    const int tail = (n_len - n_fft_frames) * n_mel;
    if (tail > 0) hipLaunchKernelGGL(k_mel_tail, dim3((tail + 255) / 256), dim3(256), 0, st, mel, n_len, n_mel, n_fft_frames, gmax);
}

void mel_batch(const MelBatch & b, int nb, int n_mel, const float * filters, const int32_t * ranges, const float * taps, hipStream_t st) {
    {
        int dev = 0; (void) hipGetDevice(&dev);
        const uint64_t bit = 1ull << (dev & 63);
        if (!(g_tables_mask.load(std::memory_order_acquire) & bit)) { upload_tables(); g_tables_mask.fetch_or(bit, std::memory_order_release); }
    }
    int n_max = 0, n_min = INT_MAX;
    for (int c = 0; c < nb; ++c) { n_max = std::max(n_max, b.n[c]); n_min = std::min(n_min, b.n[c]); }
    auto n_len = [](int n) { return (int) (((long long) n + 480000) / 160); };
    auto n_fft = [&](int n) { return std::min((n + 200) / 160 + 1, n_len(n)); };
    hipLaunchKernelGGL(k_mel_pad_b, dim3((n_max + 480400 + 255) / 256, nb), dim3(256), 0, st, b);
    hipLaunchKernelGGL(k_mel_frames_b, dim3(n_fft(n_max), nb), dim3(MEL_NT), 0, st, b, n_mel, filters, ranges, taps);
    int tail_max = 0;
    for (int c = 0; c < nb; ++c) tail_max = std::max(tail_max, (n_len(b.n[c]) - n_fft(b.n[c])) * n_mel);
    if (tail_max > 0) hipLaunchKernelGGL(k_mel_tail_b, dim3((tail_max + 255) / 256, nb), dim3(256), 0, st, b, n_mel);
    hipLaunchKernelGGL(k_mel_normalize_b, dim3((n_mel * n_len(n_max) + 255) / 256, nb), dim3(256), 0, st, b, n_mel);
}
void signal_energy_batch(const MelBatch & b, int nb, int hw, hipStream_t st) {
    int n_max = 0;
    for (int c = 0; c < nb; ++c) n_max = std::max(n_max, b.n[c]);
    if (n_max > 0) hipLaunchKernelGGL(k_signal_energy_b, dim3((n_max + 255) / 256, nb), dim3(256), 0, st, b, hw);
}

void mel_normalize(float * mel, int n, const int * gmax, hipStream_t st) {
    hipLaunchKernelGGL(k_mel_normalize, dim3((n + 255) / 256), dim3(256), 0, st, mel, n, gmax);
}

void mel_slice(const float * mel, int n_len, int n_mel, int offset, int n_frames, __half * out, int ld, int rows_total,
               hipStream_t st) {
    dim3 grid((rows_total + 31) / 32, (ld + 31) / 32);
    hipLaunchKernelGGL(k_mel_slice, grid, dim3(256), 0, st, mel, n_len, n_mel, offset, n_frames, out, ld, rows_total);
}

void mel_slice_batch(const MelSliceBatch & mb, int nb, int n_mel, int n_frames, __half * out, int ld, int rows_total, hipStream_t st) {
    dim3 grid((rows_total + 31) / 32, (ld + 31) / 32, nb);
    hipLaunchKernelGGL(k_mel_slice_batch, grid, dim3(256), 0, st, mb, n_mel, n_frames, out, ld, rows_total);
}
void fill_zero_tails(void * p, const RowLens & first_row, size_t row_bytes, size_t end_bytes, size_t stride_bytes, int count, hipStream_t st) {
    if (count <= 0 || count > 16) return;
    hipLaunchKernelGGL(k_fill_zero_tails, dim3(64, count), dim3(256), 0, st, (uint32_t *) p, first_row, row_bytes / 4, end_bytes / 4, stride_bytes / 4);
}
void fill_zero_strided(void * p, size_t bytes, size_t stride_bytes, int count, hipStream_t st) {
    if (count <= 0 || bytes == 0) return;
    hipLaunchKernelGGL(k_fill_zero_strided, dim3((unsigned) ((bytes / 4 + 255) / 256), count), dim3(256), 0, st, (uint32_t *) p, bytes / 4, stride_bytes / 4, count);
}

void signal_energy(const float * pcm, int n, int hw, float * out, float * bmin, float * bmax, hipStream_t st) {
    const int nblk = (n + 255) / 256;
    hipLaunchKernelGGL(k_signal_energy, dim3(nblk), dim3(256), 0, st, pcm, n, hw, out, bmin, bmax);
}

__device__ __forceinline__ int ts_walk(const float * __restrict__ en, const float * __restrict__ bext, int k, int bound, float th, int dir, bool above, int lane) {
    for (;;) {
        const int dist = dir > 0 ? bound - k : k - bound;
        if (dist <= 0) return k;
        const bool edge = dir > 0 ? (k & 255) == 0 : (k & 255) == 255;
        if (edge) {
            const int b = (k >> 8) + dir * lane;
            const bool inside = dir > 0 ? ((b + 1) << 8) <= bound : (b >= 0 && (b << 8) > bound);
            bool cont = false;
            if (inside) { const float e = bext[b]; cont = above ? e > th : e < th; }
            const unsigned long long m = __ballot(cont);
            const int nskip = m == ~0ull ? 64 : __builtin_ctzll(~m);
            if (nskip > 0) { k += dir * 256 * nskip; continue; }
        }
        const int to_edge = dir > 0 ? 256 - (k & 255) : (k & 255) + 1;
        int cnt = dist + 1; if (cnt > 64) cnt = 64; if (cnt > to_edge) cnt = to_edge;
        const int p = k + dir * lane;
        bool stop = false;
        if (lane < cnt) { const float x = en[p]; stop = p == bound || !(above ? x > th : x < th); }
        const unsigned long long m = __ballot(stop);
        if (m) return k + dir * __builtin_ctzll(m);
        k += dir * cnt;
    }
}

__device__ __forceinline__ float ts_trip_exact(float acc, const float (&x)[16], int n_left, int lane) {
#pragma unroll
    for (int sub = 0; sub < 4; ++sub) {
        const int b0 = sub * 256;
        if (b0 >= n_left) break;
        const uint32_t bits = __float_as_uint(acc);
        const int E = (int) ((bits >> 23) & 0xFF) - 127;
        bool done = false;
        if (b0 + 256 <= n_left && (bits >> 31) == 0 && E >= -100 && E <= 100) {
            const uint32_t units = (bits & 0x7FFFFFu) | 0x800000u;
            const float scale = __uint_as_float((uint32_t) (127 + 23 - E) << 23);
            bool bad = false; uint32_t isum = 0;
#pragma unroll
            for (int k = 0; k < 4; ++k) {
                const float tt = x[sub * 4 + k] * scale;
                const int q = __float2int_rn(tt);
                const float d = fabsf(tt - (float) q);
                bad = bad || d == 0.5f || !(tt < 8388608.0f) || tt < 0.0f;
                isum += (uint32_t) q;
            }
            if (__ballot(bad) == 0) {
                _Pragma("unroll") for (int o = 32; o > 0; o >>= 1) isum += (uint32_t) __shfl_xor((int) isum, o);
                const unsigned long long total = (unsigned long long) units + isum;
                if (total < 0x1000000ull) { acc = __uint_as_float(((uint32_t) (E + 127) << 23) | ((uint32_t) total & 0x7FFFFFu)); done = true; }
            }
        }
        if (!done) {
#pragma unroll
            for (int k = 0; k < 4; ++k) {
                const int c0 = b0 + k * 64;
                const int cnt = n_left - c0 < 64 ? n_left - c0 : 64;
                const float v = x[sub * 4 + k];
                if (cnt >= 64) {
#pragma unroll
                    for (int l = 0; l < 64; ++l) acc = acc + __builtin_bit_cast(float, __builtin_amdgcn_readlane(__builtin_bit_cast(int, v), l));
                } else {
                    for (int l = 0; l < cnt; ++l) acc = acc + __shfl(v, l);
                }
            }
        }
    }
    return acc;
}

constexpr int TS_W = 8;
__global__ __launch_bounds__(TS_W * 64) void k_ts_refine(const float * __restrict__ en_, const float * __restrict__ bmin_, const float * __restrict__ bmax_,
                                                         int n_samples_, const TsTok * __restrict__ in, TsOut * __restrict__ out) {
    __shared__ uint32_t s_sum[TS_W]; __shared__ int s_bad[TS_W]; __shared__ float s_acc;
    const int tid = threadIdx.x, lane = tid & 63, wave = tid >> 6;
    const TsTok t = in[blockIdx.x];
    const float * __restrict__ en = t.en ? t.en : en_;
    const int n_samples = t.en ? t.n_samples : n_samples_;
    const float * __restrict__ bmin = t.en ? t.en + t.ext_off : bmin_;
    const float * __restrict__ bmax = t.en ? bmin + ((size_t) t.n_samples / 256 + 2) : bmax_;
    float acc = 0.0f;
    {
        const float * p = en + t.a0;
        const int n = t.a1 - t.a0;
        auto fetch = [&](float (&dst)[16], int base) {
#pragma unroll
            for (int r = 0; r < 16; ++r) { const int e = base + r * 64 + lane; dst[r] = (e >= 0 && e < n) ? p[e] : 0.0f; }
        };
        float x[16], nx[16]; int nx_base = -1;
        int i = 0;
        while (i < n) {
            const int base = i + wave * 1024;
            if (nx_base == base) {
#pragma unroll
                for (int r = 0; r < 16; ++r) x[r] = nx[r];
            } else fetch(x, base);
            nx_base = base + TS_W * 1024;
            if (nx_base < n) fetch(nx, nx_base); else nx_base = -1;
            const uint32_t bits = __float_as_uint(acc);
            const int E = (int) ((bits >> 23) & 0xFF) - 127;
            const bool fast = (bits >> 31) == 0 && E >= -100 && E <= 100;
            bool bad = !fast || base + 1024 > n;
            uint32_t isum = 0;
            if (!bad) {
                const float scale = __uint_as_float((uint32_t) (127 + 23 - E) << 23);
#pragma unroll
                for (int r = 0; r < 16; ++r) {
                    const float tt = x[r] * scale;
                    const int q = __float2int_rn(tt);
                    const float d = fabsf(tt - (float) q);
                    bad = bad || d == 0.5f || !(tt < 8388608.0f) || tt < 0.0f;
                    isum += (uint32_t) q;
                }
                bad = bad || isum >= 0x1000000u;
                bad = __ballot(bad) != 0;
                if (!bad) { _Pragma("unroll") for (int o = 32; o > 0; o >>= 1) isum += (uint32_t) __shfl_xor((int) isum, o); }
            }
            if (lane == 0) { s_sum[wave] = isum; s_bad[wave] = bad ? 1 : 0; }
            __syncthreads();
            int k = 0;
            if (fast) {
                uint32_t running = (bits & 0x7FFFFFu) | 0x800000u;
                for (; k < TS_W; ++k) {
                    if (s_bad[k] || (unsigned long long) running + s_sum[k] >= 0x1000000ull) break;
                    running += s_sum[k];
                }
                if (k > 0) acc = __uint_as_float(((uint32_t) (E + 127) << 23) | (running & 0x7FFFFFu));
            }
            i += k * 1024;
            const bool slow = k < TS_W && i < n;
            if (slow) {
                if (wave == 0) {
                    float y[16];
                    if (k == 0) {
#pragma unroll
                        for (int r = 0; r < 16; ++r) y[r] = x[r];
                    } else fetch(y, i);
                    const float a2 = ts_trip_exact(acc, y, n - i, lane);
                    if (lane == 0) s_acc = a2;
                }
                __syncthreads();
                acc = s_acc;
                i += n - i < 1024 ? n - i : 1024;
            }
            __syncthreads();
        }
    }
    if (wave != 0) return;
    const int ns = t.a1 - t.a0;
    const float th = (float) (0.5 * (double) acc / (double) ns);
    const float x0 = en[t.s0], x1 = en[t.s1];
    const int wa = ts_walk(en, bmin, t.s0, 0, th, -1, true, lane);
    const int wb = ts_walk(en, bmax, t.s0, t.s1, th, +1, false, lane);
    const int wc = ts_walk(en, bmin, t.s1, n_samples - 1, th, +1, true, lane);
    const int wd = ts_walk(en, bmax, t.s1, 0, th, -1, false, lane);
    if (lane == 0) {
        TsOut o; o.sum = acc; o.thold = th; o.e0 = x0 > th ? 1 : 0; o.e1 = x1 > th ? 1 : 0;
        o.w_down_above_s0 = wa; o.w_up_below_s0 = wb; o.w_up_above_s1 = wc; o.w_down_below_s1 = wd;
        out[blockIdx.x] = o;
    }
}
constexpr int VB_ROW = VAD_BLOCK + 1;
__device__ __forceinline__ float vad_step(float alpha, float y, float v) { return __fmul_rn(alpha, __fsub_rn(__fadd_rn(y, v), y)); }

__global__ __launch_bounds__(64) void k_vad_blocks(const float * __restrict__ x, int n, float alpha, int warm, float * __restrict__ ys,
                                                   uint32_t * __restrict__ entry, uint32_t * __restrict__ exit_) {
    __shared__ float sx[65 * VB_ROW];
    __shared__ float sy[64 * VB_ROW];
    const int lane = threadIdx.x;
    const int t0 = blockIdx.x * (64 * VAD_BLOCK);
    for (int k = lane; k < 65 * VAD_BLOCK; k += 64) {
        const int s = t0 - VAD_BLOCK + k;
        sx[(k >> 6) * VB_ROW + (k & 63)] = (s >= 0 && s < n) ? x[s] : 0.0f;
    }
    __syncthreads();
    const int g = blockIdx.x * 64 + lane;
    const int i0 = t0 + lane * VAD_BLOCK;
    if (i0 < n) {
        const int cnt = min(VAD_BLOCK, n - i0);
        const float * own = sx + (lane + 1) * VB_ROW, * prev = sx + lane * VB_ROW;
        float * out = sy + lane * VB_ROW;
        float y; int j0 = 0;
        if (g == 0) { y = own[0]; out[0] = y; j0 = 1; }
        else {
            y = 0.0f;
            for (int j = VAD_BLOCK - warm; j < VAD_BLOCK; ++j) y = vad_step(alpha, y, prev[j]);
            entry[g] = __float_as_uint(y);
        }
        for (int j = j0; j < cnt; ++j) { y = vad_step(alpha, y, own[j]); out[j] = y; }
        exit_[g] = __float_as_uint(y);
    }
    __syncthreads();
    for (int k = lane; k < 64 * VAD_BLOCK; k += 64) {
        const int s = t0 + k;
        if (s < n) ys[s] = sy[(k >> 6) * VB_ROW + (k & 63)];
    }
}

__device__ __forceinline__ float vad_abs_sum(const float * __restrict__ p, int n, int lane) {
    auto fetch = [&](float (&dst)[16], int base) {
#pragma unroll
        for (int r = 0; r < 16; ++r) { const int e = base + r * 64 + lane; dst[r] = e < n ? fabsf(p[e]) : 0.0f; }
    };
    float acc = 0.0f, x[16], nx[16];
    if (n > 0) fetch(x, 0);
    for (int i = 0; i < n; i += 1024) {
        const bool more = i + 1024 < n;
        if (more) fetch(nx, i + 1024);
        acc = ts_trip_exact(acc, x, n - i, lane);
        if (more) {
#pragma unroll
            for (int r = 0; r < 16; ++r) x[r] = nx[r];
        }
    }
    return acc;
}

__global__ __launch_bounds__(128) void k_vad_finish(const float * __restrict__ x, float * __restrict__ ys, int n, int n_last, float alpha,
                                                    int n_blocks, const uint32_t * __restrict__ entry, const uint32_t * __restrict__ exit_,
                                                    float vad_thold, float * __restrict__ res) {
    __shared__ float s_last;
    const int tid = threadIdx.x, lane = tid & 63, wave = tid >> 6;
    int bad = 0;
    for (int b = 1 + tid; b < n_blocks; b += 128) bad |= entry[b] != exit_[b - 1];
    int rerun = 0;
    if (__syncthreads_or(bad)) {
        if (wave == 0) {
            uint32_t state = exit_[0];
            for (int b = 1; b < n_blocks; ++b) {
                if (entry[b] == state) { state = exit_[b]; continue; }
                const int i0 = b * VAD_BLOCK, cnt = min(VAD_BLOCK, n - i0);
                const float xv = lane < cnt ? x[i0 + lane] : 0.0f;
                float y = __uint_as_float(state), mine = 0.0f;
                for (int j = 0; j < cnt; ++j) {
                    y = vad_step(alpha, y, __shfl(xv, j));
                    if (lane == j) mine = y;
                }
                if (lane < cnt) ys[i0 + lane] = mine;
                state = __float_as_uint(y);
                rerun += 1;
            }
        }
        __threadfence();
        __syncthreads();
    }
    float e = 0.0f;
    if (wave == 0) e = vad_abs_sum(ys, n, lane);
    else e = vad_abs_sum(ys + (n - n_last), n_last, lane);
    if (tid == 64) s_last = e;
    __syncthreads();
    if (tid == 0) {
        float e_all = e, e_last = s_last;
        e_all /= (float) n;
        if (n_last != 0) e_last /= (float) n_last;
        const bool quiet = !(!(e_all < 0.0001f && e_last < 0.0001f) || e_last > vad_thold * e_all);
        res[0] = quiet ? 1.0f : 0.0f; res[1] = e_all; res[2] = e_last;
        ((int32_t *) res)[4] = n_blocks; ((int32_t *) res)[5] = rerun;
    }
}

size_t vad_scratch_bytes(int n) {
    const size_t nb = ((size_t) std::max(n, 0) + VAD_BLOCK - 1) / VAD_BLOCK;
    return ((size_t) std::max(n, 0) + 2 * nb + 4) * 4;
}
void vad_window_blocks(const float * x, int n, int n_last, float alpha, bool filter, float vad_thold, int warm, void * scratch, float * res,
                       hipStream_t st) {
    if (n <= 0) return;
    if (!filter) {
        hipLaunchKernelGGL(k_vad_finish, dim3(1), dim3(128), 0, st, x, const_cast<float *>(x), n, n_last, alpha, 0, nullptr, nullptr, vad_thold, res);
        return;
    }
    if (warm < 0) warm = VAD_WARM_DEFAULT;
    if (warm > VAD_BLOCK) warm = VAD_BLOCK;
    const int nb = (n + VAD_BLOCK - 1) / VAD_BLOCK;
    float * ys = (float *) scratch;
    uint32_t * entry = (uint32_t *) (ys + n), * exit_ = entry + nb;
    hipLaunchKernelGGL(k_vad_blocks, dim3((nb + 63) / 64), dim3(64), 0, st, x, n, alpha, warm, ys, entry, exit_);
    hipLaunchKernelGGL(k_vad_finish, dim3(1), dim3(128), 0, st, x, ys, n, n_last, alpha, nb, entry, exit_, vad_thold, res);
}

void ts_refine(const float * en, const float * bmin, const float * bmax, int n_samples, const TsTok * in, TsOut * out, int n_tok, hipStream_t st) {
    if (n_tok > 0) hipLaunchKernelGGL(k_ts_refine, dim3(n_tok), dim3(TS_W * 64), 0, st, en, bmin, bmax, n_samples, in, out);
}

void downmix_stereo(const float * frames, int n_frames, float * out, hipStream_t st) {
    if (n_frames > 0) hipLaunchKernelGGL(k_downmix, dim3((n_frames + 255) / 256), dim3(256), 0, st, (const float2 *) frames, n_frames, out);
}
void vad_window(const float * x, int n, int n_last, float alpha, bool filter, float vad_thold, float * res, hipStream_t st) {
    hipLaunchKernelGGL(k_vad, dim3(1), dim3(256), 0, st, x, n, n_last, alpha, filter ? 1 : 0, vad_thold, res);
}

__global__ void k_touch(int * p, int nblk) { if (threadIdx.x == 0 && blockIdx.x == 0) p[0] += 1; }
void touch(int * p, int blocks, hipStream_t st) { hipLaunchKernelGGL(k_touch, dim3(blocks), dim3(256), 0, st, p, blocks); }

static thread_local Stamp g_stamp{nullptr, 0};
void  stamp_enable(unsigned long long * base) { g_stamp.base = base; g_stamp.slot = 0; }
Stamp stamp_next() { if (!g_stamp.base) return Stamp{nullptr, 0}; return Stamp{g_stamp.base, g_stamp.slot++}; }
int   stamp_count() { return g_stamp.slot; }

void fill_zero(void * p, size_t bytes, hipStream_t st) {
    (void) hipMemsetAsync(p, 0, bytes, st);
}

}}
```

### godot-whisper_amd/csrc/kernels.h

```cpp
#pragma once
#include <memory>
#include <vector>
#include <hip/hip_runtime.h>
#include <hip/hip_fp16.h>
#include <atomic>
#include <cstdint>
#include "grammar_eval.h"

namespace wmi { namespace k {

inline void allow_full_lds(const void * kernel, std::atomic<uint64_t> & mask) {
    int dev = 0;
    (void) hipGetDevice(&dev);
    const uint64_t bit = 1ull << (dev & 63);
    if (mask.load(std::memory_order_acquire) & bit) return;
    (void) hipFuncSetAttribute(kernel, hipFuncAttributeMaxDynamicSharedMemorySize, 160 * 1024);
    mask.fetch_or(bit, std::memory_order_release);
}

#if defined(__HIPCC__)
__device__ __forceinline__ float pin_f32(float x) { asm volatile("" : "+v"(x)); return x; }
__device__ __forceinline__ __half f2h(float x) { return __float2half_rn(pin_f32(x)); }
__host__ __device__ __forceinline__ int vt_pos(int t) { return (t & ~12) | ((t & 4) << 1) | ((t & 8) >> 1); }
#endif

inline int cu_count_x8() {
    static std::atomic<int> cache[64];
    int dev = 0;
    (void) hipGetDevice(&dev);
    std::atomic<int> & c = cache[dev & 63];
    int n = c.load(std::memory_order_relaxed);
    if (n > 0) return n;
    n = 256;
    (void) hipDeviceGetAttribute(&n, hipDeviceAttributeMultiprocessorCount, dev);
    n = n > 8 ? n & ~7 : 8;
    c.store(n, std::memory_order_relaxed);
    return n;
}

#if defined(__HIPCC__)
#define WMI_ARG_NOW(x) asm volatile("" :: "s"(x))
#endif

constexpr int STAMP_WAVES = 4096;
struct Stamp { unsigned long long * base; int slot; };
void  stamp_enable(unsigned long long * base);
Stamp stamp_next();
int   stamp_count();
#if defined(__HIPCC__)
__device__ __forceinline__ unsigned long long stamp_t0(const unsigned long long * base) { return base ? wall_clock64() : 0ull; }
constexpr uint32_t STAMP_ON_BIT = 1u << 31;
__device__ __forceinline__ unsigned long long stamp_t0_if(bool on) { return on ? wall_clock64() : 0ull; }
__device__ __forceinline__ void stamp_end(unsigned long long * base, int slot, int widx, unsigned long long t0,
                                          unsigned long long tm1 = 0, unsigned long long tm2 = 0) {
    if (base && (threadIdx.x & 63) == 0 && widx < STAMP_WAVES) {
        unsigned long long * s = base + ((size_t) slot * STAMP_WAVES + widx) * 4;
        s[0] = t0; s[1] = wall_clock64(); s[2] = tm1; s[3] = tm2;
    }
}
#endif

void mel_pad(const float * pcm, int n_samples, float * pcm_pad, int n_pad_total, hipStream_t st, int * gmax_reset);
void mel_frames(const float * pcm_pad, int n_valid, int n_fft_frames, int n_len, int n_mel,
                const float * filters, const int32_t * ranges, const float * taps, float * mel, int * gmax, hipStream_t st);
void mel_normalize(float * mel, int n, const int * gmax, hipStream_t st);
struct MelBatch { const float * pcm[16]; float * pad[16]; float * mel[16]; int * gmax[16]; float * energy[16]; float * bmin[16]; float * bmax[16]; int n[16]; };
void mel_batch(const MelBatch & b, int nb, int n_mel, const float * filters, const int32_t * ranges, const float * taps, hipStream_t st);
void signal_energy_batch(const MelBatch & b, int nb, int hw, hipStream_t st);
struct MelSliceBatch { const float * mel[16]; int n_len[16]; int offset[16];
                       int n_frames[16]; };
void mel_slice_batch(const MelSliceBatch & mb, int nb, int n_mel, int n_frames, __half * out, int ld, int rows_total, hipStream_t st);
void fill_zero_strided(void * p, size_t bytes, size_t stride_bytes, int count, hipStream_t st);
struct RowLens { int n; int t[16]; };
void fill_zero_tails(void * p, const RowLens & first_row, size_t row_bytes, size_t end_bytes, size_t stride_bytes, int count, hipStream_t st);
void mel_slice(const float * mel, int n_len, int n_mel, int offset, int n_frames, __half * out, int ld,
               int rows_total, hipStream_t st);

void signal_energy(const float * pcm, int n, int hw, float * out, float * bmin, float * bmax, hipStream_t st);
struct TsTok { int32_t s0, s1, a0, a1;
               const float * en; int32_t n_samples, ext_off; };
struct TsOut { float sum, thold; int32_t e0, e1;
               int32_t w_down_above_s0, w_up_below_s0, w_up_above_s1, w_down_below_s1; };
void ts_refine(const float * en, const float * bmin, const float * bmax, int n_samples, const TsTok * in, TsOut * out, int n_tok, hipStream_t st);

void downmix_stereo(const float * frames, int n_frames, float * out, hipStream_t st);
void vad_window(const float * x, int n, int n_last, float alpha, bool filter, float vad_thold, float * res, hipStream_t st);
constexpr int VAD_BLOCK = 64, VAD_WARM_DEFAULT = 32;
size_t vad_scratch_bytes(int n);
void vad_window_blocks(const float * x, int n, int n_last, float alpha, bool filter, float vad_thold, int warm, void * scratch, float * res,
                       hipStream_t st);

struct Stepper;
struct ResamplePlan {
    int error = 0;
    int converter = 2;
    long long n_out = 0, n_used = 0;
    int half_len = 0, index_inc = 0, increment = 0;
    double float_inc = 0.0, out_scale = 0.0;
    bool need_table = false;
    std::shared_ptr<Stepper> stepper;
};
bool sinc_table(int converter, const float ** coeffs, int * count, int * increment);
ResamplePlan resample_plan(long long n_in, long long out_cap, double ratio, int converter);
void resample_table(const ResamplePlan & pl, const int ** pos, const double ** frac);
void resample_positions(const ResamplePlan & pl, long long n, long long * pos, double * frac);
void resample_launch(const ResamplePlan & pl, const float * d_in, long long n_in, float * d_out, const float * d_coeffs,
                     const int * d_pos, const double * d_frac, hipStream_t st);
void resample_launch_stereo(const ResamplePlan & pl, const float * d_frames_xy, long long n_in, float * d_out, const float * d_coeffs,
                            const int * d_pos, const double * d_frac, long long first, hipStream_t st);
long long resample_first_dirty(const ResamplePlan & old_pl, long long n_old, const ResamplePlan & new_pl);
enum SrcKind : int { SRC_F32_MONO = 0, SRC_F32_STEREO = 1, SRC_S16_MONO = 2, SRC_S16_STEREO = 3, SRC_S8_MONO = 4, SRC_S8_STEREO = 5 };
void resample_launch_kind(const ResamplePlan & pl, int kind, const void * d_src, long long n_in, float * d_out, const float * d_coeffs,
                          const int * d_pos, const double * d_frac, long long first, hipStream_t st);

bool wav_decode(int kind, const void * d_src, long long n_frames, float * out, hipStream_t st);
long long channel_bins_count(long long n, long long rate);
bool channel_bins(int kind, const void * d_src, long long n, long long rate, void * d_bins, hipStream_t st);

enum Epi : int {
    EPI_F16_BIAS = 0,
    EPI_F16_BIAS_GELU,
    EPI_F32_BIAS_RESID,
    EPI_CONV2,
    EPI_QKV_ENC,
    EPI_QKV_DEC,
    EPI_CROSS_KV,
    EPI_Q_SCALED,
};
struct GemmArgs {
    const __half * A;  int lda;
    const __half * W;  int ldw;
    int M, N, K;
    const float * bias;
    void *  C;   int ldc;
    const float * resid; int ldr;
    void *  aux; int ldaux;
    void *  aux2; int ldaux2;
    float   scale;
    int     S;
    int64_t layer_stride;
    int     rows_per_chunk;
    int     conv2_out_rows;
    int64_t chunk_stride_aux2;
    int     no_glds;
    unsigned long long * probe;
};
void gemm(int epi, const GemmArgs & a, hipStream_t st);
struct GemmLogEntry { int epi, M, N, K; size_t off; int cap; };
struct GemmLog { unsigned long long * buf = nullptr; size_t cap_words = 0, used = 0; std::vector<GemmLogEntry> entries; };
void gemm_log_install(GemmLog * log);
bool gemm8(int epi, int bm, bool swapped, const GemmArgs & a, hipStream_t st, int ks = 64);

enum GemmOrient : int {
    GEMM_ORIENT_ROWS = 0,
    GEMM_ORIENT_COLS = 1,
    GEMM_ORIENT_PER_TILE = 2,
};
struct GemmPlan {
    int epi = 0;
    int kernel = 0;
    int bm = 0, bn = 0;
    int waves = 0;
    int ring = 0, ring_w = 0;
    int dma = 0;
    int orient = 0;
    int ks = 0;
// ... 254 lines not shown
```

### godot-whisper_amd/csrc/wmi.h

```cpp
#pragma once

#include <hip/hip_runtime.h>
#include <hip/hip_fp16.h>

#include <cmath>
#include <cstdint>
#include <cstdio>
#include <map>
#include <functional>
#include <mutex>
#include <random>
#include <set>
#include <string>
#include <vector>

#include "../../include/whisper_mi355.h"
#include "../../include/wmi_device.h"
#include "kernels.h"

namespace wmi {

void log_msg(ggml_log_level lvl, const char * fmt, ...) __attribute__((format(printf, 2, 3)));
#define WMI_ERR(...)  ::wmi::log_msg(GGML_LOG_LEVEL_ERROR, __VA_ARGS__)
#define WMI_WARN(...) ::wmi::log_msg(GGML_LOG_LEVEL_WARN,  __VA_ARGS__)
// ... 72 lines not shown
    std::vector<EncLayerW> enc;
    const float  *e_ln_g, *e_ln_b;
    const __half *w_ckv;   const float *b_ckv;
    k::QMat       q_ckv;
    const float  *d_pe;
    const __half *d_te;
    k::QMat       q_te;
    int           qtype = 0;
    size_t        matrix_bytes = 0;
    std::vector<DecLayerW> dec;
    const float  *d_ln_g, *d_ln_b;
    const float  *mel_filters;
    const float   *mel_taps;
    const int32_t *mel_ranges;
};

bool upload_weights(const ModelFile & mf, const uint8_t * host_buf, Weights & w, hipStream_t st);
bool plan_weights(const ModelFile & mf, Weights & w);
void free_weights(Weights & w);

struct KVCell { int32_t pos = -1; std::set<int32_t> seq; bool has(int32_t s) const { return seq.count(s) != 0; } };
struct KVCache {
    uint32_t head = 0, size = 0, n = 0;
    std::vector<KVCell> cells;
    __half * k = nullptr;  __half * v = nullptr;
};
struct Batch {
    std::vector<int32_t> token, pos, seq_id; std::vector<int8_t> logits;
    int n_tokens = 0;
    void prep_legacy(const int32_t * tokens, int n, int n_past, int seq);
};
bool  kv_find_slot(KVCache & c, const Batch & b);
int   kv_cell_max(const KVCache & c);
void  kv_clear(KVCache & c);
void  kv_seq_rm(KVCache & c, int32_t seq, int32_t p0, int32_t p1);
void  kv_seq_cp(KVCache & c, int32_t src, int32_t dst, int32_t p0, int32_t p1);

struct Sequence {
    std::vector<whisper_token_data> tokens;
    int    result_len = 0;
    double sum_logprobs_all = 0, sum_logprobs = 0, avg_logprobs = 0, entropy = 0, score = 0;
};
struct PartialUtf8 { uint32_t value = 0; int n_remain = 0; };
struct GrammarPos  { int rule, off; };
struct Grammar {
    std::vector<std::vector<whisper_grammar_element>> rules;
    std::vector<std::vector<GrammarPos>> stacks;
    PartialUtf8 partial;
};
struct Decoder {
    Sequence sequence;
    Grammar  grammar;
    int  i_batch = 0, seek_delta = 0;
    bool failed = false, completed = false, has_ts = false;
    std::vector<float> probs, logits, logprobs;
    std::mt19937 rng{0};
};
struct Segment {
    int64_t t0, t1; std::string text; std::vector<whisper_token_data> tokens; bool speaker_turn_next;
    std::vector<int64_t> t_dtw; int32_t i_tok0 = 0;
};

struct Mel { int n_len = 0, n_len_org = 0, n_mel = 0; };
enum { WINDOW_EMITTED = 0, WINDOW_DROPPED = 1, WINDOW_GATED = 2 };
struct WindowRec { int32_t seek = 0; float p = -1.0f; int32_t outcome = WINDOW_EMITTED, seg0 = 0, n_seg = 0; };

struct DeviceState {
    hipStream_t stream = nullptr; bool stream_own_queue = false;
    float * pcm = nullptr;      size_t pcm_cap = 0;
    float * mel = nullptr;      size_t mel_cap = 0;
    float * mel_max = nullptr;
    const float * last_pcm = nullptr; int last_pcm_n = 0;
    struct WavJob * pcm_job = nullptr;
    float * energy = nullptr;   size_t energy_cap = 0;
    float * energy_host = nullptr;
    size_t  energy_dev_cap = 0;
    hipStream_t copy_stream = nullptr; hipEvent_t energy_ev = nullptr;
    hipEvent_t ph_ev[4] = {nullptr, nullptr, nullptr, nullptr}; bool ph_mel = false, ph_enc = false; int64_t ph_host0 = 0;
    hipStream_t energy_wait_stream = nullptr;
    hipStream_t mel_stream = nullptr;  hipEvent_t mel_ev = nullptr;
    bool    energy_pending = false;
    bool    energy_device_only = false;
    void *  ts_host = nullptr;
    __half * mel_t = nullptr;
    __half * conv1 = nullptr;
    float  * x     = nullptr;
    float  * embd_conv = nullptr;
    __half * xn    = nullptr;
    __half * q     = nullptr, * k = nullptr;
    __half * vt    = nullptr;
    __half * att   = nullptr;
    __half * h     = nullptr;
    float  * rowmax = nullptr;
    int8_t * aq = nullptr;  float * ads = nullptr;  int aq_rows = 0;
    __half * aq16 = nullptr, * wq16 = nullptr; size_t wq16_elems = 0;
    float  * att32 = nullptr;
    float  * datt32 = nullptr;
    float  * enc_out = nullptr;
    __half * enc_out_h = nullptr;
    __half * kvc_k = nullptr, * kvc_v = nullptr;
    int      Tpad = 0;
    int      conv1_max_T = 0;
    int32_t * d_tokens = nullptr, * d_pos = nullptr;
    float   * d_mask = nullptr;
    int32_t * d_rows = nullptr;
    float  * dx = nullptr;  __half * dxn = nullptr, * dq = nullptr, * datt = nullptr, * dh = nullptr;
    float  * xattn = nullptr;
    float  * logits = nullptr;  int logits_rows_cap = 0;
    void   * pinned = nullptr;  size_t pinned_bytes = 0;
    void   * step_dev = nullptr;   void * step_host = nullptr;
    void   * sample_dev = nullptr; void * sample_host = nullptr;
    void   * filter_scratch = nullptr;
    uint8_t * ban_dev = nullptr;   uint64_t ban_sig = ~0ull;
    void * mlp_hand = nullptr; unsigned long long * mlp_arrive = nullptr;
    bool pair_off = false; int pair_backoff = 0;
    int  pair_fallbacks = 0, pair_slow_events = 0;
    struct StepGraph { hipGraph_t graph = nullptr; hipGraphExec_t exec = nullptr; int T = -1; int seen = 0; };
    StepGraph step_graphs[8];
    bool chain_valid = false; int32_t chain_token = 0, chain_pos = 0, chain_head = 0;
    int32_t step_seq = 0;
    bool    keep_logits_on_device = false;
    void  * draw_host = nullptr;
    void  * draw_scratch = nullptr;
    bool    step_capture_failed = false;
    struct GrammarBufs {
        uint8_t * vbytes = nullptr; uint32_t * voff = nullptr; char * rules = nullptr; size_t rules_cap = 0; int n_rules = 0, n_elems = 0;
        ge::RowState * states = nullptr; uint8_t * reject = nullptr; void * scratch = nullptr; void * host = nullptr;
    } gram;
    void  * nsp_scratch = nullptr; float * nsp_logits = nullptr; void * nsp_host = nullptr; int32_t nsp_seq = 0; int nsp_row = -1;
    int     step_seen_T = -1;
    k::AlignBufs dtw{}; size_t dtw_cap[7] = {}; void * dtw_host = nullptr; int32_t dtw_seq = 0;
    bool dtw_collect = false, dtw_active = false; int dtw_n_sot = 0, dtw_M = 0;
    int dec_n = 0;
    struct ScoreReq { const int32_t * item_row = nullptr; int n_items = 0; const int32_t * d_target = nullptr, * d_place = nullptr;
                      void * staging = nullptr; size_t staging_bytes = 0; float * logits_out = nullptr; const int32_t * place = nullptr; };
    void * score_scratch = nullptr; int32_t * score_items = nullptr; size_t score_items_cap = 0; float * score_lp = nullptr; size_t score_lp_cap = 0;
    void * score_host = nullptr; size_t score_host_cap = 0; int32_t score_seq = 0;
    const ScoreReq * score_req = nullptr;
    struct DraftReq { const k::DecStep * d_steps = nullptr; const int32_t * d_targets = nullptr; int n_targets = 0; k::FsPartial * part = nullptr;
                      k::SampleOut * out_host = nullptr; int32_t * d_match = nullptr; float * logits_out = nullptr; mutable int nsp_flag = -1; };
    void * draft_part = nullptr, * draft_dev = nullptr, * draft_host = nullptr; int draft_cap = 0; int32_t draft_seq = 0;
    const DraftReq * draft_req = nullptr;
};

struct State {
    std::recursive_mutex mu;
    int     device = 0;
    int64_t t_sample_us = 0, t_encode_us = 0, t_decode_us = 0, t_batchd_us = 0, t_prompt_us = 0, t_mel_us = 0;
    int32_t n_sample = 0, n_encode = 0, n_decode = 0, n_batchd = 0, n_prompt = 0, n_fail_p = 0, n_fail_h = 0;
    KVCache kv_self;
    Mel     mel;
    Batch   batch;
    Decoder decoders[8];
    std::vector<float> logits;
    std::vector<Segment> result_all;
    std::vector<WindowRec> windows;
    struct DtwDims { int n = 0, n_sot = 0, R = 0, M = 0, n_pairs = 0; } dtw_last; std::vector<int32_t> dtw_jumps;
    int64_t t_dtw_us = 0; int32_t n_dtw = 0;
    int64_t t_score_us = 0; int32_t n_score = 0, n_score_launches = 0;
    std::vector<int32_t> draft; struct wmi_draft_status draft_status{0, 0, 0, 0, 1}; float * draft_logits_out = nullptr; int draft_logits_cap = 0;
    int32_t gram_steps_dev = 0, gram_rows_host = 0; float gram_reject_us = 0.0f;
    std::vector<int32_t> dtw_pairs_call;
    std::vector<int32_t> prompt_past;
    int     lang_id = 0;
    std::vector<float> lang_probs;
    int64_t t_beg = 0, t_last = 0; int32_t tid_last = 0;
// ... 129 lines not shown
template <typename BUFS> inline k::Q8Rows q8_rows(const BUFS & d, int K) {
    return k::Q8Rows{d.aq, d.ads, d.ads + (size_t) (K / 32) * d.aq_rows, d.aq_rows, d.aq16, d.wq16, d.wq16_elems};
}
bool encode_layers_q(whisper_context & ctx, int T);
struct EncBufsQ {
    int T, nb, Tpad;
    float * x; __half * q, * k, * vt, * h; float * att32; float * enc_out; __half * enc_out_h; __half * kvc_k, * kvc_v;
    k::Q8Rows A, A4;
    int P; k::RowLens lens;
};
bool encode_layers_q_on(whisper_context & ctx, const EncBufsQ & e, hipStream_t s);
void enqueue_rows_step_q(whisper_context & ctx, int nb);
void enqueue_rows_lang_step_q(whisper_context & ctx, int nb, float * out);
bool decode_layers_q(whisper_context & ctx, int n, int n_kv, int kv_head, int Tc, const std::vector<int> & rows, float * lang_out = nullptr,
                     const int32_t * nsp_row_dev = nullptr, float * nsp_logits = nullptr, const DeviceState::ScoreReq * score = nullptr,
                     const DeviceState::DraftReq * draft = nullptr);
void enqueue_greedy_step_q(whisper_context & ctx, int Tc);
struct GrammarFlat { std::vector<ge::Elem> elems; std::vector<uint32_t> rule_off; bool ok = false; };
GrammarFlat grammar_flatten(const Grammar & g);
bool grammar_row_state(const Grammar & g, const GrammarFlat & f, ge::RowState & out);
void grammar_vocab_flat(const Vocab & v, std::vector<uint8_t> & bytes, std::vector<uint32_t> & off);
bool grammar_eval_host(const GrammarFlat & f, const std::vector<uint8_t> & bytes, const std::vector<uint32_t> & off, const ge::RowState & st,
                       uint8_t * mask, int n_vocab);
void grammar_reject_mask(const whisper_context & ctx, const Grammar & g, uint8_t * mask);
struct StepFilter { bool ban_blank, last_ts, penult_ts; int ts_floor_end, ts_initial_start; };
inline StepFilter make_step_filter(const Vocab & v, const HParams & hp, const whisper_full_params & params, const Decoder & d) {
    const auto & h = d.sequence.tokens;
    StepFilter f{};
    const bool initial = h.empty();
    f.ban_blank = params.suppress_blank && initial;
    f.last_ts = !h.empty() && h.back().id >= v.beg;
    f.penult_ts = h.size() < 2 || h[h.size() - 2].id >= v.beg;
    f.ts_floor_end = d.has_ts ? v.beg + d.seek_delta / 2 : v.beg;
    f.ts_initial_start = v.n_vocab;
    if (initial && params.max_initial_ts > 0.0f) {
        const float precision = float(WHISPER_CHUNK_SIZE) / hp.n_audio_ctx;
        f.ts_initial_start = v.beg + (int) std::round(params.max_initial_ts / precision) + 1;
    }
    return f;
}
void decoder_advance(const whisper_context & ctx, const whisper_full_params & params, Decoder & d, int i, int seek, int seek_end, int n_max);
struct DraftPlan { int n = 0; std::vector<StepFilter> filters; };
DraftPlan draft_plan(const whisper_context & ctx, const whisper_full_params & params, int P, const int32_t * draft, int n_offered, int seek, int seek_end);
bool draft_group(whisper_context & ctx, const DeviceState::DraftReq & rq, int r0, int nr);
bool draft_verify(whisper_context & ctx, const std::vector<int32_t> & prompt, const int32_t * draft, const DraftPlan & plan, int nsp_row,
                  float * logits_out, std::vector<whisper_token_data> & picks, int & accepted);
enum : unsigned { STEP_FORM_LONG_KV = 1, STEP_FORM_CHAINED = 2, STEP_FORM_GRAPH = 4, STEP_FORM_PAIRED = 8, STEP_FORM_FRONTED = 16,
                  STEP_FORM_BACKED = 32, STEP_FORM_RERUN = 64, STEP_FORM_SLOW = 128, STEP_FORM_QUANTISED = 256,
                  STEP_FORM_JOINED = 512 };
bool decode_greedy_step(whisper_context & ctx, int32_t token, int32_t pos, const StepFilter & f, whisper_token_data & out, unsigned * forms = nullptr);
bool upload_static_ban(whisper_context & ctx, const whisper_full_params & params);
bool no_speech_ensure(whisper_context & ctx, DeviceState & d);
bool no_speech_from_logits(whisper_context & ctx, const float * logits, int row);
bool no_speech_from_row(whisper_context & ctx, const float * x);
bool no_speech_read(State & st, float * p);
enum { NSP_EMIT = 0, NSP_FALLBACK = 1, NSP_DROP = 2, NSP_GATE = 3 };
int  no_speech_rule(int mode, float p, float thold, bool failed, double avg_logprob, float logprob_thold);
std::vector<int32_t> dtw_default_pairs(const HParams & hp);
bool dtw_ensure(DeviceState & d, int nh, int n, int R, int M, int n_pairs);
bool dtw_layer(whisper_context & ctx, int il, int n, int Tc);
bool dtw_window(whisper_context & ctx, const std::vector<int32_t> & x, int n_sot, int M);
void dtw_path_host(int R, int M, const float * A, int32_t * jumps, int32_t * path, int * n_path);
struct ScorePass { int c0 = 0, c1 = 0; std::vector<int32_t> token, pos, seq, target, place; std::vector<int8_t> flag; };
struct ScorePlan { std::vector<int32_t> prefix, first, prefix_target; std::vector<ScorePass> passes; };
int  score_plan(const Vocab & v, const HParams & hp, size_t kv_cells, const wmi_score_params & p, const int32_t * tokens, const int32_t * n_tokens, int n_texts, ScorePlan & out);
bool score_group(whisper_context & ctx, const DeviceState::ScoreReq & rq, int r0, int nr, int & item);
int  score_texts(whisper_context & ctx, const wmi_score_params & p, const int32_t * tokens, const int32_t * n_tokens, int n_texts, wmi_text_score * out,
                 float * token_logprobs, float * logits_out);
bool sample_rows_device(whisper_context & ctx, const StepFilter * f, const int * rows, int n_rows, float temperature, int k,
                        const double * u, int tid_default, whisper_token_data * out);
bool grammar_device_begin(whisper_context & ctx, const GrammarFlat & gf);
bool sample_rows_grammar_device(whisper_context & ctx, const GrammarFlat & gf, const Grammar * const * gr, float penalty, const StepFilter * f,
                                const int * rows, int n_rows, float temperature, int k, bool best, const double * u, int tid_default,
                                whisper_token_data * out);
bool wait_for_sample(const k::SampleOut * r, int32_t want, hipStream_t s, int32_t * status = nullptr);
void pool_run(int n_tasks, const std::function<void(int)> & fn);
double bench_greedy_step_chain(whisper_context & ctx, int iters);
double bench_rows_step_chain(whisper_context & ctx, int nb, int iters);
int    step_stamps(whisper_context & ctx, double * out, int cap, bool chained);
struct BusyScope { int dev; bool counted; explicit BusyScope(int device); ~BusyScope(); };
int busy_transcriptions(int device);
bool signal_energy_device(whisper_context & ctx, int hw, bool sync = true, int via_dma = 0);
bool ts_refine_device(State & st, const k::TsTok * in, int n, k::TsOut * out);
struct TsRef { State * st; int seg, j; };
bool flush_token_timestamps(whisper_context & ctx, State & st);
bool flush_token_timestamps_of(whisper_context & ctx, const std::vector<State *> & states);
bool signal_energy_wait(State & st);

void process_logits(whisper_context & ctx, Decoder & dec, const whisper_full_params & params, float temperature);
whisper_token_data sample_token(whisper_context & ctx, Decoder & dec, bool best);
std::vector<whisper_token_data> sample_token_topk(whisper_context & ctx, Decoder & dec, int k, bool count = true);
void sequence_score(const whisper_full_params & params, Sequence & seq);
Grammar grammar_init(const whisper_grammar_element ** rules, size_t n_rules, size_t i_start_rule);
void grammar_penalise(const whisper_context & ctx, const Grammar & g, float penalty, std::vector<float> & logits);
void grammar_accept_token(const whisper_context & ctx, Grammar & g, int32_t token);
std::vector<int32_t> tokenize(const Vocab & vocab, const std::string & text);
int  lang_auto_detect(whisper_context & ctx, int offset_ms, float * lang_probs);
int  lang_detect_head(whisper_context & ctx, int offset_ms, float * lang_probs, bool defer = false);
int  lang_probs_from_logits(const float * logits, float * lang_probs);
int  full(whisper_context & ctx, whisper_full_params params, const float * samples, const float * d_samples, int n_samples);
int  check_audio_ctxs(const whisper_context & ctx, const int * audio_ctx, int n, const char * who);
int  lockstep_sets(const int * eff_T, int n, bool quantised, bool per_row, int * order, int * set_of);
int  full_batch(whisper_context & ctx, whisper_full_params params, const float * const * pcm, const int * n_samples, int n_chunks, bool on_device,
                const int * audio_ctx = nullptr);
void free_batch(whisper_context & ctx);
void frame_energy_host(const float * x, int n, float * e);
wmi_long_params long_default_params();
bool long_params_ok(const wmi_long_params & p);
int  long_window(int n_samples, int offset_ms, int duration_ms, int * f0, int * f1, int * n_sub);
int  long_plan(const float * e, int F, int n, const wmi_long_params & lp, int n_audio_ctx, std::vector<wmi_long_piece> & out);
void free_long(BatchWork & w);
int  ensure_replicas(whisper_context & ctx, int n);
void trim_replicas(whisper_context & ctx, int keep);
void emit_window(whisper_context & ctx, State & st, const whisper_full_params & params, int seek, const std::vector<int32_t> & prompt,
                 size_t n_prompt_init, const Decoder & best);
std::vector<float> signal_energy(const float * signal, int n_samples, int hw);
void token_level_timestamps(whisper_context & ctx, State & st, int i_segment, float thold_pt, float thold_ptsum);
float seq_sum_f32(const float * p, int n);
int  wrap_segment(whisper_context & ctx, State & st, int max_len, bool split_on_word);

int         lang_id(const char * lang);
const char *lang_str(int id);
const char *lang_str_full(int id);
int         lang_max_id();
int         lang_count();

}
```

### godot-whisper_amd/runtime.py

```python
from __future__ import annotations

import ctypes as C
import os
import pathlib

import numpy as np

from . import abi

LIB_PATH = pathlib.Path(__file__).resolve().parent / "libwhisper_mi355.so"
if os.environ.get("WMI_LIB_PATH"):
    LIB_PATH = pathlib.Path(os.environ["WMI_LIB_PATH"]).resolve()

DEVICE_API = [
    ("wmi_device_count", C.c_int, []),
    ("wmi_version", C.c_char_p, []),
    ("wmi_init_from_buffer_on_device", C.c_void_p, [C.c_void_p, C.c_size_t, C.c_int]),
    ("wmi_init_host_only", C.c_void_p, [C.c_void_p, C.c_size_t]),
    ("wmi_pcm_to_mel_device", C.c_int, [C.c_void_p, C.c_void_p, C.c_int]),
    ("wmi_full_device_pcm", C.c_int, [C.c_void_p, abi.whisper_full_params, C.c_void_p, C.c_int, C.POINTER(C.c_float)]),
    ("wmi_full_batch", C.c_int, [C.c_void_p, abi.whisper_full_params, C.POINTER(C.c_void_p), C.POINTER(C.c_int), C.c_int, C.c_int]),
    ("wmi_full_batch_ctx", C.c_int, [C.c_void_p, abi.whisper_full_params, C.POINTER(C.c_void_p), C.POINTER(C.c_int), C.POINTER(C.c_int),
                                     C.c_int, C.c_int]),
    ("wmi_batch_enc_dims", C.c_int, [C.c_void_p, C.POINTER(C.c_int), C.POINTER(C.c_int), C.POINTER(C.c_int)]),
    ("wmi_set_lockstep_exact", None, [C.c_int]),
    ("wmi_batch_select", C.c_int, [C.c_void_p, C.c_int]),
    ("wmi_batch_chunk_mode", C.c_int, [C.c_void_p, C.c_int]),
    ("wmi_batch_lang_id", C.c_int, [C.c_void_p, C.c_int]),
    ("wmi_batch_lang_probs", C.c_int, [C.c_void_p, C.c_int, C.POINTER(C.c_float)]),
    ("wmi_lang_detect", C.c_int, [C.c_void_p, C.c_int, C.POINTER(C.c_float)]),
    ("wmi_selftest_lang_probs", C.c_int, [C.POINTER(C.c_float), C.POINTER(C.c_float)]),
    ("wmi_set_batch_replicas", C.c_int, [C.c_void_p, C.c_int]),
    ("wmi_set_lockstep_groups", C.c_int, [C.c_void_p, C.c_int]),
    ("wmi_selftest_pool", C.c_int64, [C.c_int, C.c_int]),
    ("wmi_selftest_seqsum", C.c_int, [C.POINTER(C.c_float), C.c_int, C.POINTER(C.c_float), C.POINTER(C.c_float)]),
    ("wmi_get_batch_timings", None, [C.c_void_p, C.POINTER(C.c_int64), C.POINTER(C.c_int32)]),
    ("wmi_set_audio_ctx", C.c_int, [C.c_void_p, C.c_int]),
    ("wmi_get_tensor", C.c_int, [C.c_void_p, C.c_char_p, C.POINTER(C.c_float), C.c_int]),
    ("wmi_mel_dims", C.c_int, [C.c_void_p, C.POINTER(C.c_int), C.POINTER(C.c_int), C.POINTER(C.c_int)]),
    ("wmi_get_timings", None, [C.c_void_p, C.POINTER(C.c_int64), C.POINTER(C.c_int32)]),
    ("wmi_stream", C.c_void_p, [C.c_void_p]),
    ("wmi_process_logits", C.c_int, [C.c_void_p, abi.whisper_full_params, C.POINTER(C.c_float), C.POINTER(C.c_int32),
                                      C.c_int, C.c_int, C.c_int, C.c_float, C.POINTER(C.c_float),
                                      C.POINTER(C.c_float), C.POINTER(C.c_float)]),
    ("wmi_sample_draws", C.c_int, [C.c_void_p, C.POINTER(C.c_float), C.POINTER(C.c_float), C.c_int, C.c_int,
                                    C.POINTER(abi.whisper_token_data)]),
    ("wmi_selftest_proj", C.c_double, [C.c_void_p, C.c_int, C.c_int, C.c_int]),
    ("wmi_selftest_greedy_step", C.c_int, [C.c_void_p, C.c_int32, C.c_int, C.POINTER(C.c_float), C.POINTER(abi.whisper_token_data),
                                           C.POINTER(C.c_int)]),
    ("wmi_selftest_filters", C.c_int, [C.c_void_p, abi.whisper_full_params, C.c_int, C.c_int, C.c_void_p, C.c_void_p, C.c_void_p, C.c_void_p,
                                       C.c_void_p, C.c_float, C.c_void_p, C.c_void_p, C.c_int, C.c_void_p, C.c_void_p, C.c_int, C.c_int,
                                       C.c_void_p]),
    ("wmi_bench_kernel", C.c_double, [C.c_void_p, C.c_int, C.c_int]),
    ("wmi_reload_knobs", None, []),
    ("wmi_pair_status", C.c_int, [C.c_void_p, C.POINTER(C.c_int32), C.c_int]),
    ("wmi_step_stamps", C.c_int, [C.c_void_p, C.POINTER(C.c_double), C.c_int, C.c_int]),
    ("wmi_encoder_gemm_stamps", C.c_int, [C.c_void_p, C.c_int, C.POINTER(C.c_double), C.c_int]),
    ("wmi_pool_init", C.c_void_p, [C.c_void_p, C.c_size_t, C.POINTER(C.c_int), C.c_int]),
    ("wmi_pool_free", None, [C.c_void_p]),
    ("wmi_pool_size", C.c_int, [C.c_void_p]),
    ("wmi_pool_context", C.c_void_p, [C.c_void_p, C.c_int]),
    ("wmi_pool_full", C.c_int, [C.c_void_p, abi.whisper_full_params, C.POINTER(C.c_void_p), C.POINTER(C.c_int), C.c_int]),
    ("wmi_pool_select", C.c_void_p, [C.c_void_p, C.c_int]),
    ("wmi_pool_device_time_us", C.c_int64, [C.c_void_p, C.c_int]),
    ("wmi_downmix_stereo", C.c_int, [C.c_void_p, C.c_void_p, C.c_int, C.c_int, C.c_void_p]),
    ("wmi_vad", C.c_int, [C.c_void_p, C.c_void_p, C.c_int, C.c_int, C.c_float, C.c_float, C.c_void_p]),
    ("wmi_selftest_ts_refine", C.c_int, [C.c_void_p, C.c_void_p, C.c_int, C.c_void_p, C.c_int, C.c_void_p, C.c_void_p, C.c_void_p]),
    ("wmi_selftest_resample_plan", C.c_int, [C.c_int, C.c_int, C.c_int, C.c_int, C.c_void_p, C.c_void_p, C.c_void_p, C.c_int, C.c_void_p,
                                             C.c_void_p]),
    ("wmi_resample", C.c_int, [C.c_void_p, C.c_void_p, C.c_int, C.c_int, C.c_int, C.c_int, C.c_int, C.c_void_p, C.c_int]),
    ("wmi_capture_init", C.c_void_p, [C.c_void_p, C.c_int, C.c_int, C.c_int]),
    ("wmi_capture_free", None, [C.c_void_p]),
    ("wmi_capture_push", C.c_int, [C.c_void_p, C.c_void_p, C.c_int, C.c_int]),
    ("wmi_capture_keep_last", C.c_int, [C.c_void_p, C.c_int]),
    ("wmi_capture_resample", C.c_int, [C.c_void_p, C.POINTER(C.c_int)]),
    ("wmi_capture_pcm", C.c_void_p, [C.c_void_p, C.POINTER(C.c_int)]),
    ("wmi_capture_read_pcm", C.c_int, [C.c_void_p, C.c_void_p, C.c_int]),
    ("wmi_capture_vad", C.c_int, [C.c_void_p, C.c_float, C.c_float, C.c_void_p]),
    ("wmi_capture_full", C.c_int, [C.c_void_p, abi.whisper_full_params]),
    ("wmi_capture_full_batch", C.c_int, [C.POINTER(C.c_void_p), C.c_int, abi.whisper_full_params, C.POINTER(C.c_int)]),
    ("wmi_capture_stats", C.c_int, [C.c_void_p, C.POINTER(C.c_int64)]),
    ("wmi_selftest_capture_plan", C.c_int, [C.c_int, C.c_int, C.c_int, C.c_int, C.POINTER(C.c_longlong), C.POINTER(C.c_longlong),
                                            C.POINTER(C.c_longlong)]),
    ("wmi_selftest_vad", C.c_int, [C.c_void_p, C.c_void_p, C.c_int, C.c_int, C.c_int, C.c_float, C.c_float, C.c_int, C.c_int, C.c_void_p,
                                   C.c_void_p]),
    ("wmi_model_header", C.c_size_t, [C.c_void_p, C.c_size_t, C.c_void_p, C.c_size_t]),
    ("wmi_arena_ptr", C.c_void_p, [C.c_void_p]),
    ("wmi_init_from_header", C.c_void_p, [C.c_void_p, C.c_size_t, C.c_int]),
    ("wmi_arena_commit", C.c_int, [C.c_void_p]),
    ("wmi_weights_pending", C.c_int, [C.c_void_p]),
    ("wmi_weights_bytes", C.c_size_t, [C.c_void_p, C.c_int]),
    ("wmi_selftest_quant", C.c_int, [C.c_int, C.c_int, C.c_int, C.c_void_p, C.c_void_p, C.c_void_p, C.c_int, C.c_int, C.c_int,
                                     C.c_void_p, C.c_void_p, C.c_void_p]),
    ("wmi_selftest_attn_encoder", C.c_int, [C.c_int, C.c_int, C.c_int, C.c_int, C.c_int, C.c_int, C.c_int, C.c_int, C.c_void_p, C.c_int, C.c_int,
                                            C.c_int, C.c_void_p, C.c_void_p, C.c_void_p, C.c_uint32, C.c_void_p]),
    ("wmi_selftest_qkv_encoder", C.c_int, [C.c_int, C.c_int, C.c_int, C.c_int, C.c_int, C.c_void_p, C.c_void_p, C.c_void_p, C.c_uint32, C.c_int,
                                           C.c_void_p, C.c_void_p, C.c_void_p]),
    ("wmi_selftest_attn_decoder", C.c_int, [C.c_int, C.c_int, C.c_int, C.c_int, C.c_int, C.c_int, C.c_int, C.c_void_p, C.c_void_p, C.c_int, C.c_int,
                                            C.c_int, C.c_void_p, C.c_void_p, C.c_void_p, C.c_uint32, C.c_int, C.c_void_p]),
    ("wmi_selftest_attn_cross", C.c_int, [C.c_int, C.c_int, C.c_int, C.c_int, C.c_int, C.c_int, C.c_int, C.c_int, C.c_void_p, C.c_int, C.c_int,
                                          C.c_void_p, C.c_float, C.c_void_p, C.c_void_p, C.c_uint32, C.c_int, C.c_void_p, C.c_void_p, C.c_void_p,
                                          C.c_void_p, C.c_void_p]),
    ("wmi_selftest_gemm_plan", C.c_int, [C.c_int, C.c_int, C.c_int, C.c_int, C.c_int, C.c_int, C.c_void_p]),
    ("wmi_selftest_gemm", C.c_int, [C.c_int, C.c_int, C.c_int, C.c_int, C.c_int, C.c_int, C.c_int, C.c_float, C.c_int, C.c_int, C.c_int, C.c_int,
                                    C.c_int, C.c_int, C.c_int, C.c_void_p, C.c_void_p, C.c_void_p, C.c_void_p, C.c_uint32, C.c_int, C.c_void_p,
                                    C.c_void_p, C.c_void_p, C.c_void_p]),
    ("wmi_selftest_qkv_encoder_q", C.c_int, [C.c_int, C.c_int, C.c_int, C.c_int, C.c_int, C.c_int, C.c_void_p, C.c_void_p, C.c_void_p, C.c_uint32,
                                             C.c_int, C.c_void_p, C.c_void_p, C.c_void_p]),
    ("wmi_selftest_lockstep_sets", C.c_int, [C.POINTER(C.c_int), C.c_int, C.c_int, C.c_int, C.POINTER(C.c_int), C.POINTER(C.c_int)]),
    ("wmi_set_no_speech", C.c_int, [C.c_void_p, C.c_int]),
    ("wmi_full_n_windows", C.c_int, [C.c_void_p]),
    ("wmi_full_get_window", C.c_int, [C.c_void_p, C.c_int, C.POINTER(abi.wmi_window)]),
    ("wmi_full_get_segment_no_speech_prob", C.c_float, [C.c_void_p, C.c_int]),
    ("wmi_full_n_windows_from_state", C.c_int, [C.c_void_p]),
    ("wmi_full_get_window_from_state", C.c_int, [C.c_void_p, C.c_int, C.POINTER(abi.wmi_window)]),
    ("wmi_full_get_segment_no_speech_prob_from_state", C.c_float, [C.c_void_p, C.c_int]),
    ("wmi_selftest_no_speech_rule", C.c_int, [C.c_int, C.c_float, C.c_float, C.c_int, C.c_double, C.c_float]),
    ("wmi_selftest_no_speech", C.c_int, [C.c_int, C.c_int, C.c_int, C.c_int, C.c_int, C.c_void_p, C.c_void_p, C.c_void_p, C.c_int,
                                         C.c_void_p, C.c_void_p]),
    ("wmi_set_token_dtw", C.c_int, [C.c_void_p, C.c_int, C.POINTER(C.c_int32), C.c_int]),
    ("wmi_token_dtw_heads", C.c_int, [C.c_void_p, C.POINTER(C.c_int32), C.c_int]),
    ("wmi_full_get_token_dtw", C.c_int64, [C.c_void_p, C.c_int, C.c_int]),
    ("wmi_full_get_token_dtw_from_state", C.c_int64, [C.c_void_p, C.c_int, C.c_int]),
    ("wmi_token_dtw_dims", C.c_int, [C.c_void_p] + [C.POINTER(C.c_int)] * 5),
    ("wmi_get_token_dtw_timings", None, [C.c_void_p, C.POINTER(C.c_int64), C.POINTER(C.c_int32)]),
    ("wmi_selftest_dtw_matrix", C.c_int, [C.c_int] * 8 + [C.c_void_p, C.c_void_p, C.c_void_p, C.c_int, C.c_void_p]),
    ("wmi_selftest_dtw_path", C.c_int, [C.c_int, C.c_int, C.c_int, C.c_void_p, C.c_void_p, C.c_void_p, C.POINTER(C.c_int)]),
    ("wmi_set_grammar_device", C.c_int, [C.c_void_p, C.c_int]),
    ("wmi_grammar_status", C.c_int, [C.c_void_p, C.POINTER(abi.wmi_grammar_status)]),
    ("wmi_selftest_grammar", C.c_int, [C.c_void_p, abi.whisper_full_params, C.c_int, C.c_int, C.c_void_p, C.c_void_p, C.c_void_p, C.c_void_p]),
    ("wmi_selftest_grammar_sample", C.c_int, [C.c_void_p, abi.whisper_full_params, C.c_int, C.c_int, C.c_void_p, C.c_void_p, C.c_void_p,
                                              C.c_void_p, C.c_void_p, C.c_float, C.c_void_p, C.c_int, C.c_int, C.c_void_p]),
    ("wmi_score_default_params", abi.wmi_score_params, []),
    ("wmi_score_texts", C.c_int, [C.c_void_p, abi.wmi_score_params, C.c_void_p, C.c_void_p, C.c_int, C.POINTER(abi.wmi_text_score), C.c_void_p]),
    ("wmi_score_texts_with_state", C.c_int, [C.c_void_p, C.c_void_p, abi.wmi_score_params, C.c_void_p, C.c_void_p, C.c_int,
                                             C.POINTER(abi.wmi_text_score), C.c_void_p, C.c_void_p]),
    ("wmi_score_pcm", C.c_int, [C.c_void_p, abi.wmi_score_params, C.c_void_p, C.c_int, C.c_int, C.c_int, C.c_void_p, C.c_void_p, C.c_int,
                                C.POINTER(abi.wmi_text_score), C.c_void_p]),
    ("wmi_get_score_timings", None, [C.c_void_p, C.POINTER(C.c_int64), C.POINTER(C.c_int32), C.POINTER(C.c_int32)]),
    ("wmi_selftest_score_rows", C.c_int, [C.c_int, C.c_int, C.c_int, C.c_void_p, C.c_void_p, C.c_void_p]),
    ("wmi_selftest_score_plan", C.c_int, [C.c_void_p, abi.wmi_score_params, C.c_void_p, C.c_void_p, C.c_int, C.c_void_p, C.c_int,
                                          C.POINTER(C.c_int), C.c_void_p, C.c_void_p, C.c_void_p, C.c_int, C.POINTER(C.c_int), C.c_void_p, C.c_int]),
    ("wmi_set_draft", C.c_int, [C.c_void_p, C.c_void_p, C.c_int]),
    ("wmi_set_draft_with_state", C.c_int, [C.c_void_p, C.c_void_p, C.c_void_p, C.c_int]),
    ("wmi_draft_status", C.c_int, [C.c_void_p, C.POINTER(abi.wmi_draft_status)]),
    ("wmi_draft_status_from_state", C.c_int, [C.c_void_p, C.POINTER(abi.wmi_draft_status)]),
    ("wmi_capture_set_draft", C.c_int, [C.c_void_p, C.c_int]),
    ("wmi_selftest_draft_plan", C.c_int, [C.c_void_p, abi.whisper_full_params, C.c_void_p, C.c_int, C.c_void_p, C.c_int, C.POINTER(C.c_int32),
                                          C.c_void_p, C.c_void_p]),
    ("wmi_selftest_draft_rows", C.c_int, [C.c_int, C.c_int, C.c_int, C.c_void_p, C.c_void_p, C.c_void_p, C.c_void_p, C.c_void_p,
# ... 74 lines not shown
```

### include/wmi_device.h

```cpp
#ifndef WMI_DEVICE_H
#define WMI_DEVICE_H

#include <stddef.h>
#include <stdint.h>

#include "whisper_mi355.h"

#ifdef __cplusplus
extern "C" {
#endif

WHISPER_API int          wmi_device_count(void);
WHISPER_API const char * wmi_version(void);

WHISPER_API struct whisper_context * wmi_init_from_buffer_on_device(const void * buffer, size_t buffer_size, int device);

WHISPER_API struct whisper_context * wmi_init_host_only(const void * buffer, size_t buffer_size);

WHISPER_API size_t wmi_model_header(const void * model, size_t model_size, void * out, size_t cap);
WHISPER_API void * wmi_arena_ptr(struct whisper_context * ctx);
WHISPER_API struct whisper_context * wmi_init_from_header(const void * header, size_t header_size, int device);
WHISPER_API int    wmi_arena_commit(struct whisper_context * ctx);
WHISPER_API int    wmi_weights_pending(struct whisper_context * ctx);
WHISPER_API size_t wmi_weights_bytes(struct whisper_context * ctx, int which);
// ... 3 lines not shown
WHISPER_API int wmi_full_device_pcm(struct whisper_context * ctx, struct whisper_full_params params,
                                    const float * d_samples, int n_samples, const float * h_samples_for_timestamps);

struct wmi_pool;
WHISPER_API struct wmi_pool * wmi_pool_init(const void * model, size_t model_size, const int * devices, int n_devices);
WHISPER_API void wmi_pool_free(struct wmi_pool * pool);
WHISPER_API int  wmi_pool_size(struct wmi_pool * pool);
WHISPER_API struct whisper_context * wmi_pool_context(struct wmi_pool * pool, int i);
WHISPER_API int  wmi_pool_full(struct wmi_pool * pool, struct whisper_full_params params, const float * const * pcm,
                               const int * n_samples, int n_chunks);
WHISPER_API struct whisper_context * wmi_pool_select(struct wmi_pool * pool, int chunk);
WHISPER_API int64_t wmi_pool_device_time_us(struct wmi_pool * pool, int i);

WHISPER_API int wmi_downmix_stereo(struct whisper_context * ctx, const float * frames, int n_frames, int on_device, float * mono_out);

WHISPER_API int wmi_resample(struct whisper_context * ctx, const float * src, int n_frames, int src_rate, int dst_rate, int converter,
                             int on_device, float * dst, int dst_capacity);
WHISPER_API int wmi_vad(struct whisper_context * ctx, const float * pcm, int n_samples, int on_device, float vad_thold, float freq_thold,
                        float * energies);

struct wmi_capture;
WHISPER_API struct wmi_capture * wmi_capture_init(struct whisper_context * ctx, int mix_rate, int converter, int frames_hint);
WHISPER_API void          wmi_capture_free(struct wmi_capture * cap);
WHISPER_API int           wmi_capture_push(struct wmi_capture * cap, const float * frames_xy, int n_frames, int on_device);
WHISPER_API int           wmi_capture_keep_last(struct wmi_capture * cap, int n_frames);
WHISPER_API int           wmi_capture_resample(struct wmi_capture * cap, int * expected);
WHISPER_API const float * wmi_capture_pcm(struct wmi_capture * cap, int * n_samples);
WHISPER_API int           wmi_capture_read_pcm(struct wmi_capture * cap, float * dst, int capacity);
WHISPER_API int           wmi_capture_vad(struct wmi_capture * cap, float vad_thold, float freq_thold, float * energies);
WHISPER_API int           wmi_capture_full(struct wmi_capture * cap, struct whisper_full_params params);
WHISPER_API int           wmi_capture_stats(struct wmi_capture * cap, int64_t * out4);
WHISPER_API int           wmi_capture_full_batch(struct wmi_capture * const * caps, int n, struct whisper_full_params params, const int * audio_ctx);
WHISPER_API int wmi_selftest_capture_plan(int n_old, int n_new, int src_rate, int converter, long long * first_dirty,
                                          long long * n_out_old, long long * n_out_new);
WHISPER_API int wmi_selftest_vad(struct whisper_context * ctx, const float * pcm, int n, int sample_rate, int last_ms, float vad_thold,
                                 float freq_thold, int form, int warm, float * energies, int32_t * stats2);

WHISPER_API int wmi_full_batch(struct whisper_context * ctx, struct whisper_full_params params, const float * const * pcm,
                               const int * n_samples, int n_chunks, int pcm_on_device);
WHISPER_API int wmi_full_batch_ctx(struct whisper_context * ctx, struct whisper_full_params params, const float * const * pcm,
                                   const int * n_samples, const int * audio_ctx, int n_chunks, int pcm_on_device);
WHISPER_API int wmi_selftest_lockstep_sets(const int * audio_ctx, int n, int n_audio_ctx, int quantised, int * order, int * set_of);
WHISPER_API int wmi_batch_enc_dims(struct whisper_context * ctx, int * rows, int * row_period, int * row_T);
WHISPER_API void wmi_set_lockstep_exact(int on);
WHISPER_API int wmi_batch_select(struct whisper_context * ctx, int chunk);
WHISPER_API int wmi_batch_chunk_mode(struct whisper_context * ctx, int chunk);
WHISPER_API int wmi_batch_lang_id(struct whisper_context * ctx, int chunk);
WHISPER_API int wmi_batch_lang_probs(struct whisper_context * ctx, int chunk, float * probs100);

WHISPER_API int wmi_lang_detect(struct whisper_context * ctx, int offset_ms, float * lang_probs);
WHISPER_API int wmi_set_lockstep_groups(struct whisper_context * ctx, int n);

WHISPER_API int wmi_set_batch_replicas(struct whisper_context * ctx, int n);

WHISPER_API void wmi_get_batch_timings(struct whisper_context * ctx, int64_t * t4, int32_t * n_steps);

WHISPER_API int wmi_set_audio_ctx(struct whisper_context * ctx, int n_audio_ctx);

WHISPER_API int wmi_get_tensor(struct whisper_context * ctx, const char * name, float * dst, int n);
WHISPER_API int wmi_mel_dims(struct whisper_context * ctx, int * n_len, int * n_len_org, int * n_mel);

WHISPER_API void wmi_get_timings(struct whisper_context * ctx, int64_t * t6, int32_t * n5);

WHISPER_API void * wmi_stream(struct whisper_context * ctx);

WHISPER_API int wmi_process_logits(struct whisper_context * ctx, struct whisper_full_params params, const float * raw_logits,
                                   const whisper_token * hist, int n_hist, int has_ts, int seek_delta, float temperature,
                                   float * out_logits, float * out_logprobs, float * out_probs);
WHISPER_API int wmi_sample_draws(struct whisper_context * ctx, const float * probs, const float * logprobs, int n_draw,
                                 int reseed, whisper_token_data * out);

WHISPER_API double wmi_selftest_proj(struct whisper_context * ctx, int op, int n, int layer);

WHISPER_API int wmi_selftest_greedy_step(struct whisper_context * ctx, whisper_token token, int pos, float * logits, whisper_token_data * out,
                                         int * forms);

WHISPER_API int wmi_selftest_filters(struct whisper_context * ctx, struct whisper_full_params params, int mode, int n_rows,
                                     const float * logits, const whisper_token * hist, const int * n_hist, const int * has_ts,
                                     const int * seek_delta, float temperature, const void * W, const float * x, int K, float * logits_out,
                                     const double * u, int k, int tid_default, whisper_token_data * out);

WHISPER_API int wmi_selftest_ts_refine(struct whisper_context * ctx, const float * envelope, int n, const int * s0s1, int n_tok,
                                       float * sums, float * thold, int * walks);
WHISPER_API int wmi_selftest_resample_plan(int n_frames, int src_rate, int dst_rate, int converter, long long * frames_gen,
                                           long long * frames_used, int * closed_form, int n_pos, long long * pos, double * frac);

WHISPER_API int wmi_selftest_quant(int device, int qtype, int mode, const void * w_blocks, const float * x, const int32_t * tokens,
                                   int M, int N, int K, float * out, int8_t * out_qs, float * out_ds);

WHISPER_API int wmi_selftest_attn_encoder(int device, int B, int T, int Tpad, int S, int H, int qk_rows, int out_rows, const int32_t * row_T,
                                          int want_f32, int form, int groups, const uint16_t * q, const uint16_t * k, const uint16_t * v,
                                          uint32_t sentinel, void * out);
WHISPER_API int wmi_selftest_qkv_encoder(int device, int M, int S, int Tpad, int rows_per_chunk, const uint16_t * xn, const uint16_t * W,
                                         const float * bias, uint32_t sentinel, int out_rows, uint16_t * q, uint16_t * k, uint16_t * vt);
WHISPER_API int wmi_selftest_attn_decoder(int device, int form, int n, int S, int H, int cap, int cache_rows, const int32_t * n_kv, const float * mask,
                                          int via_dev, int long_cache, int want_f32, const uint16_t * q, const uint16_t * kc, const uint16_t * vc,
                                          uint32_t sentinel, int out_rows, void * out);
WHISPER_API int wmi_selftest_attn_cross(int device, int form, int consumer, int n, int S, int H, int T, int kv_rows, const int32_t * row_lens,
                                        int want_f32, int lanes, const void * q, float qscale, const uint16_t * kc, const uint16_t * vc,
                                        uint32_t sentinel, int out_rows, void * out, float * pmax, float * part_l, float * part_o, int * info);
WHISPER_API int wmi_selftest_gemm_plan(int epi, int M, int N, int K, int S, int n_cu, int * out);
WHISPER_API int wmi_selftest_gemm(int device, int epi, int M, int N, int K, int lda, int S, float scale, int n_layers, int rows_per_chunk,
                                  int conv2_out_rows, int Tpad, int ld_pad, int in_place, int force8_bm, const uint16_t * A,
                                  const uint16_t * W, const float * bias, const float * resid, uint32_t sentinel, int out_rows, void * C,
                                  void * aux, void * aux2, int * plan_out);
WHISPER_API int wmi_selftest_qkv_encoder_q(int device, int qtype, int M, int S, int Tpad, int rows_per_chunk, const float * x,
                                           const void * w_blocks, const float * bias, uint32_t sentinel, int out_rows, uint16_t * q,
                                           uint16_t * k, uint16_t * vt);

WHISPER_API double wmi_bench_kernel(struct whisper_context * ctx, int which, int iters);

WHISPER_API void wmi_reload_knobs(void);

WHISPER_API int wmi_pair_status(struct whisper_context * ctx, int32_t * out3, int rearm);

WHISPER_API int wmi_step_stamps(struct whisper_context * ctx, double * out, int cap, int chained);

WHISPER_API int wmi_encoder_gemm_stamps(struct whisper_context * ctx, int chunks, double * out, int cap);

WHISPER_API int wmi_selftest_seqsum(const float * x, int n, float * out_blocked, float * out_plain);
WHISPER_API int wmi_selftest_lang_probs(const float * logits100, float * probs100);

struct wmi_window {
    int32_t seek;
    float   no_speech_prob;
    int32_t outcome;
    int32_t i_segment;
    int32_t n_segments;
};
WHISPER_API int   wmi_set_no_speech(struct whisper_context * ctx, int mode);
WHISPER_API int   wmi_full_n_windows(struct whisper_context * ctx);
WHISPER_API int   wmi_full_get_window(struct whisper_context * ctx, int i, struct wmi_window * out);
WHISPER_API float wmi_full_get_segment_no_speech_prob(struct whisper_context * ctx, int i_segment);
WHISPER_API int   wmi_full_n_windows_from_state(struct whisper_state * state);
WHISPER_API int   wmi_full_get_window_from_state(struct whisper_state * state, int i, struct wmi_window * out);
WHISPER_API float wmi_full_get_segment_no_speech_prob_from_state(struct whisper_state * state, int i_segment);
WHISPER_API int   wmi_selftest_no_speech_rule(int mode, float p, float thold, int failed, double avg_logprob, float logprob_thold);
WHISPER_API int   wmi_selftest_no_speech(int device, int form, int rows, int n_vocab, int nosp, const float * logits, const uint16_t * W,
                                         const float * x, int K, float * logits_out, float * p_out);

WHISPER_API int     wmi_set_token_dtw(struct whisper_context * ctx, int mode, const int32_t * layer_head, int n_pairs);
WHISPER_API int     wmi_token_dtw_heads(struct whisper_context * ctx, int32_t * layer_head, int cap);
WHISPER_API int64_t wmi_full_get_token_dtw(struct whisper_context * ctx, int i_segment, int i_token);
WHISPER_API int64_t wmi_full_get_token_dtw_from_state(struct whisper_state * state, int i_segment, int i_token);
WHISPER_API int     wmi_token_dtw_dims(struct whisper_context * ctx, int * n, int * n_sot, int * R, int * M, int * n_pairs);
WHISPER_API void    wmi_get_token_dtw_timings(struct whisper_context * ctx, int64_t * us, int32_t * n_windows);
WHISPER_API int     wmi_selftest_dtw_matrix(int device, int L, int S, int H, int n, int n_sot, int M, int T, const uint16_t * q, const uint16_t * k,
                                            const int32_t * layer_head, int n_pairs, float * A_out);
WHISPER_API int     wmi_selftest_dtw_path(int device, int R, int M, const float * A, int32_t * jumps, int32_t * path, int * n_path);

struct wmi_grammar_status {
    int32_t steps_device;
    int32_t rows_host;
    int32_t cap_stacks;
    int32_t cap_depth;
    int32_t cap_words;
    float   reject_us;
};
WHISPER_API int wmi_set_grammar_device(struct whisper_context * ctx, int mode);
WHISPER_API int wmi_grammar_status(struct whisper_context * ctx, struct wmi_grammar_status * out);
WHISPER_API int wmi_selftest_grammar(struct whisper_context * ctx, struct whisper_full_params params, int where, int n_rows,
                                     const whisper_token * hist, const int * n_hist, uint8_t * reject_out, uint32_t * overflow_out);
WHISPER_API int wmi_selftest_grammar_sample(struct whisper_context * ctx, struct whisper_full_params params, int mode, int n_rows,
                                            const float * logits, const whisper_token * hist, const int * n_hist, const int * has_ts,
                                            const int * seek_delta, float temperature, const double * u, int k, int tid_default,
                                            whisper_token_data * out);
// ... 111 lines not shown
```

Before: 10850 x realtime.

## Poll a host-mapped completion word for token-timestamp refine and restructure the kernel

Replaces the hipStreamSynchronize after the token-timestamp refine kernel with a bounded host spin on a pinned completion word. The last block of the grid writes that word after an atomic counter reaches the grid size. The kernel is also restructured: it uses vectorized float4 fetches and a one-pass scan-based exact summation. Its four envelope walks now run on separate waves instead of all on wave 0, and the edge-skip walk checks 256 blocks per ballot round instead of 64. The envelope is requested via a DMA path and the host wait on the envelope is skipped when it stays device-only. Together these aim to cut host sync latency and the kernel's serial critical path, at the cost of a busy-wait CPU spin and much more intricate summation code that must stay bit-exact.

```diff
diff --git a/godot-whisper_amd/csrc/api.cpp b/godot-whisper_amd/csrc/api.cpp
--- a/godot-whisper_amd/csrc/api.cpp
+++ b/godot-whisper_amd/csrc/api.cpp
@@ -418,6 +418,8 @@
     } catch (...) { WMI_ERR("wmi_resample: out of memory\n"); return -3; }
 }
 
+int wmi_selftest_ts_poll_us(int us) { return ts_poll_bound_us(us); }
+
 int wmi_selftest_ts_refine(struct whisper_context * ctx, const float * envelope, int n, const int * s0s1, int n_tok, float * sums, float * thold, int * walks) {
     if (!ctx || !envelope || n <= 0 || !s0s1 || n_tok <= 0 || n_tok > 4096 || !sums || !thold || !walks) return -1;
     CtxScope lk(ctx);
@@ -427,8 +429,9 @@
         const size_t nb = (size_t) n / 256 + 2;
         std::vector<float> ext(2 * nb, 0.0f);
         for (size_t b = 0; b * 256 < (size_t) n; ++b) {
-            float lo = INFINITY, hi = -INFINITY;
-            for (size_t i = b * 256; i < std::min<size_t>((b + 1) * 256, (size_t) n); ++i) { lo = std::min(lo, envelope[i]); hi = std::max(hi, envelope[i]); }
+            float lo = INFINITY, hi = -INFINITY; bool nan = false;
+            for (size_t i = b * 256; i < std::min<size_t>((b + 1) * 256, (size_t) n); ++i) { lo = std::min(lo, envelope[i]); hi = std::max(hi, envelope[i]); nan = nan || envelope[i] != envelope[i]; }
+            if (nan) lo = hi = NAN;
             ext[b] = lo; ext[nb + b] = hi;
         }
         std::vector<k::TsTok> in(n_tok);
diff --git a/godot-whisper_amd/csrc/batch.cpp b/godot-whisper_amd/csrc/batch.cpp
--- a/godot-whisper_amd/csrc/batch.cpp
+++ b/godot-whisper_amd/csrc/batch.cpp
@@ -45,6 +45,7 @@
     dfree(d.pcm); dfree(d.mel); dfree(d.mel_max); dfree(d.energy);
     if (d.energy_host) (void) hipHostFree(d.energy_host);
     if (d.ts_host) (void) hipHostFree(d.ts_host);
+    dfree(d.ts_count);
     delete st;
 }
 
@@ -864,7 +865,7 @@
         const int ng = std::min(group, n_chunks - g0);
         if (!lang_known) for (int r = 0; r < ng; ++r) if (n_samples[g0 + r] <= 0) { WMI_ERR("%s: failed to auto-detect language (chunk %d is empty)\n", __func__, g0 + r); return -3; }
         std::vector<Row> rows(ng);
-        static const bool ts_device = !(getenv("WMI_TS_DEVICE") && atoi(getenv("WMI_TS_DEVICE")) == 0);
+        const bool ts_device = ts_device_enabled();
         static const bool mel_per_chunk = getenv("WMI_MEL_PER_CHUNK") != nullptr;
         const bool env_batched = params.token_timestamps && ts_device;
         const bool mel_batched = !mel_per_chunk && ng >= 2 && (env_batched || !params.token_timestamps);
diff --git a/godot-whisper_amd/csrc/device.cpp b/godot-whisper_amd/csrc/device.cpp
--- a/godot-whisper_amd/csrc/device.cpp
+++ b/godot-whisper_amd/csrc/device.cpp
@@ -167,6 +167,7 @@
     if (d.mel_ev) { (void) hipEventDestroy(d.mel_ev); d.mel_ev = nullptr; }
     dfree(d.energy); if (d.energy_host) (void) hipHostFree(d.energy_host);
     if (d.ts_host) (void) hipHostFree(d.ts_host);
+    dfree(d.ts_count);
     dfree(d.pcm); dfree(d.mel); dfree(d.mel_max); dfree(d.mel_t); dfree(d.conv1); dfree(d.x); dfree(d.embd_conv);
     dfree(d.xn); dfree(d.q); dfree(d.k); dfree(d.vt); dfree(d.att); dfree(d.h); dfree(d.rowmax); dfree(d.enc_out);
     dfree(d.enc_out_h); dfree(d.d_tokens); d.d_pos = nullptr; d.d_mask = nullptr; d.d_rows = nullptr; dfree(d.dx); dfree(d.dxn);
@@ -357,20 +358,61 @@
     return sync ? signal_energy_wait(st) : true;
 }
 
+bool ts_device_enabled() {
+    static const bool on = !(getenv("WMI_TS_DEVICE") && atoi(getenv("WMI_TS_DEVICE")) == 0);
+    return on;
+}
+
+static std::atomic<int> g_ts_poll_us{2000000};
+int ts_poll_bound_us(int us) { return g_ts_poll_us.exchange(us < 0 ? 0 : us); }
+
+hipStream_t envelope_stream_of(const State & st) { return envelope_stream(st.dev); }
+
 bool ts_refine_device(State & st, const k::TsTok * in, int n, k::TsOut * out) {
     DeviceState & d = st.dev;
     constexpr int CAP = 448;
     if (n <= 0) return true;
     hipStream_t es = envelope_stream(d);
     if (n > CAP || !d.energy || !es) return false;
-    if (!d.ts_host && !HIP_OK(hipHostMalloc(&d.ts_host, CAP * (sizeof(k::TsTok) + sizeof(k::TsOut)), hipHostMallocDefault))) return false;
+    if (!d.ts_host) {
+        if (!HIP_OK(hipHostMalloc(&d.ts_host, CAP * (sizeof(k::TsTok) + sizeof(k::TsOut)) + 64, hipHostMallocDefault))) return false;
+        memset(d.ts_host, 0, CAP * (sizeof(k::TsTok) + sizeof(k::TsOut)) + 64);
+    }
+    if (!d.ts_count) {
+        if (!dalloc(d.ts_count, 1)) return false;
+        HIP_TRY(hipMemsetAsync(d.ts_count, 0, sizeof(int), es));
+    }
     k::TsTok * hin = (k::TsTok *) d.ts_host; k::TsOut * hout = (k::TsOut *) (hin + CAP);
+    const volatile int32_t * word = (const volatile int32_t *) (hout + CAP);
     memcpy(hin, in, (size_t) n * sizeof(k::TsTok));
     const size_t nb = (size_t) d.last_pcm_n / 256 + 2;
-    k::ts_refine(d.energy, d.energy + d.energy_cap, d.energy + d.energy_cap + nb, d.last_pcm_n, hin, hout, n, es);
-    HIP_TRY(hipStreamSynchronize(es));
+    d.ts_seq = d.ts_seq >= 0x7fffffff ? 1 : d.ts_seq + 1;
+    k::ts_refine(d.energy, d.energy + d.energy_cap, d.energy + d.energy_cap + nb, d.last_pcm_n, hin, hout, n, es, d.ts_count, (int32_t *) word, d.ts_seq);
+    if (hipGetLastError() != hipSuccess) return false;
+    bool seen = false;
+    const int bound = g_ts_poll_us.load(std::memory_order_relaxed);
+    if (bound > 0) {
+        const int64_t tb = time_us();
+        for (uint32_t it = 1;; ++it) {
+            if (*word == d.ts_seq) { seen = true; break; }
+            __builtin_ia32_pause();
+            if ((it & 0x3FF) == 0 && time_us() - tb > bound) break;
+        }
+    }
+    if (!seen) HIP_TRY(hipStreamSynchronize(es));
+    asm volatile("" ::: "memory");
     memcpy(out, hout, (size_t) n * sizeof(k::TsOut));
-    return true;
+    if (d.energy_device_only) d.energy_pending = false;
+    return true;
+}
+
+bool signal_energy_ready(State & st) {
+    DeviceState & d = st.dev;
+    if (d.energy_pending && d.energy_device_only) {
+        st.energy = nullptr; st.energy_bmin = st.energy_bmax = nullptr; st.energy_n = d.last_pcm_n; st.energy_on_device = true;
+        return true;
+    }
+    return signal_energy_wait(st);
 }
 
 bool signal_energy_wait(State & st) {
diff --git a/godot-whisper_amd/csrc/full.cpp b/godot-whisper_amd/csrc/full.cpp
--- a/godot-whisper_amd/csrc/full.cpp
+++ b/godot-whisper_amd/csrc/full.cpp
@@ -41,7 +41,7 @@
     st.result_all.push_back(std::move(seg));
     int n_new = 1;
     if (params.token_timestamps) {
-        (void) signal_energy_wait(st);
+        (void) signal_energy_ready(st);
         token_level_timestamps(ctx, st, (int) st.result_all.size() - 1, params.thold_pt, params.thold_ptsum);
         if (params.max_len > 0) n_new = wrap_segment(ctx, st, params.max_len, params.split_on_word);
     }
@@ -146,7 +146,7 @@
 
     if (params.token_timestamps) {
         st.t_beg = 0; st.t_last = 0; st.tid_last = 0;
-        if (n_samples > 0 && !signal_energy_device(ctx, 32, false)) { WMI_ERR("%s: failed to compute the signal envelope\n", __func__); return -2; }
+        if (n_samples > 0 && !signal_energy_device(ctx, 32, false, ts_device_enabled() ? 3 : 0)) { WMI_ERR("%s: failed to compute the signal envelope\n", __func__); return -2; }
     }
 
     const int seek_start = params.offset_ms / 10;
@@ -711,6 +711,7 @@
     std::vector<State *> involved;
     for (State * s : states) if (s && !s->ts_pending.empty()) { if (!first) first = s; involved.push_back(s); ts_collect(ctx, *s, in, ref); }
     if (!first || in.empty()) return true;
+    for (State * s : involved) if (s != first && envelope_stream_of(*s) != envelope_stream_of(*first)) (void) signal_energy_wait(*s);
     std::vector<k::TsOut> res(in.size());
     for (size_t q0 = 0; q0 < in.size(); q0 += 448) {
         const int cnt = (int) std::min<size_t>(448, in.size() - q0);
diff --git a/godot-whisper_amd/csrc/k_mel.hip b/godot-whisper_amd/csrc/k_mel.hip
--- a/godot-whisper_amd/csrc/k_mel.hip
+++ b/godot-whisper_amd/csrc/k_mel.hip
@@ -467,12 +467,20 @@
         if (dist <= 0) return k;
         const bool edge = dir > 0 ? (k & 255) == 0 : (k & 255) == 255;
         if (edge) {
-            const int b = (k >> 8) + dir * lane;
-            const bool inside = dir > 0 ? ((b + 1) << 8) <= bound : (b >= 0 && (b << 8) > bound);
-            bool cont = false;
-            if (inside) { const float e = bext[b]; cont = above ? e > th : e < th; }
-            const unsigned long long m = __ballot(cont);
-            const int nskip = m == ~0ull ? 64 : __builtin_ctzll(~m);
+            bool cont[4];
+#pragma unroll
+            for (int j = 0; j < 4; ++j) {
+                const int b = (k >> 8) + dir * (lane + 64 * j);
+                const bool inside = dir > 0 ? ((b + 1) << 8) <= bound : (b >= 0 && (b << 8) > bound);
+                cont[j] = false;
+                if (inside) { const float e = bext[b]; cont[j] = above ? e > th : e < th; }
+            }
+            int nskip = 0;
+#pragma unroll
+            for (int j = 0; j < 4; ++j) {
+                const unsigned long long m = __ballot(cont[j]);
+                if (nskip == 64 * j) nskip += m == ~0ull ? 64 : __builtin_ctzll(~m);
+            }
             if (nskip > 0) { k += dir * 256 * nskip; continue; }
         }
         const int to_edge = dir > 0 ? 256 - (k & 255) : (k & 255) + 1;
@@ -531,9 +539,101 @@
 }
 
 constexpr int TS_W = 8;
+constexpr uint32_t TS_BAD = 0xFFFFFFFFu, TS_TOP = 0x1000000u;
+__device__ __forceinline__ float ts_uniform(float v) { return __uint_as_float((uint32_t) __builtin_amdgcn_readfirstlane((int) __float_as_uint(v))); }
+__device__ __forceinline__ bool ts_fast(uint32_t bits) { const int E = (int) ((bits >> 23) & 0xFF) - 127; return (bits >> 31) == 0 && E >= -100 && E <= 100; }
+__device__ __forceinline__ bool ts_units(float x, float scale, uint32_t & q) {
+    const float tt = x * scale;
+    const int qi = __float2int_rn(tt);
+    q = (uint32_t) qi;
+    return fabsf(tt - (float) qi) == 0.5f || !(tt < 8388608.0f) || tt < 0.0f;
+}
+__device__ __forceinline__ void ts_scan(const float (&x)[16], int start, float scale, int lane, uint32_t & s, int & fb, uint32_t & ex, uint32_t & total) {
+    s = 0; fb = 16;
+    bool open = true;
+#pragma unroll
+    for (int r = 0; r < 16; ++r) {
+        uint32_t q; const bool flag = ts_units(x[r], scale, q);
+        if (lane * 16 + r >= start && open) { if (flag) { fb = r; open = false; } else s += q; }
+    }
+    s = s < TS_TOP ? s : TS_TOP;
+    uint32_t inc = s;
+#pragma unroll
+    for (int o = 1; o < 64; o <<= 1) { const uint32_t v = (uint32_t) __shfl_up((int) inc, o); if (lane >= o) inc += v; }
+    ex = inc - s; total = (uint32_t) __shfl((int) inc, 63);
+}
+__device__ __forceinline__ float ts_plain_lanes(float acc, const float (&x)[16], int l0, int l1, int start) {
+    for (int l = l0; l < l1; ++l) {
+#pragma unroll
+        for (int r = 0; r < 16; ++r) {
+            const float v = __builtin_bit_cast(float, __builtin_amdgcn_readlane(__builtin_bit_cast(int, x[r]), l));
+            if (l * 16 + r >= start) acc = __fadd_rn(acc, v);
+        }
+    }
+    return acc;
+}
+__device__ __forceinline__ float ts_trip_onepass(float acc, const float (&x)[16], int lane, bool scanned, uint32_t s, int fb, uint32_t ex) {
+    int start = 0, lane0 = 0;
+    uint32_t off = 0;
+    while (start < 1024) {
+        acc = ts_uniform(acc);
+        const uint32_t bits = __float_as_uint(acc);
+        if (bits == 0u) {
+            int r0 = 16; float xs = 0.0f;
+#pragma unroll
+            for (int r = 15; r >= 0; --r) if (lane * 16 + r >= start && __float_as_uint(x[r]) != 0u) { r0 = r; xs = x[r]; }
+            const unsigned long long m = __ballot(r0 < 16);
+            if (!m) return acc;
+            const int L = __builtin_ctzll(m);
+            acc = __fadd_rn(0.0f, __shfl(xs, L));
+            start = __builtin_amdgcn_readfirstlane(L * 16 + __shfl(r0, L) + 1);
+            scanned = false;
+            continue;
+        }
+        if (!ts_fast(bits)) {
+            for (int l = start >> 4; l < 64; ++l) {
+                acc = ts_plain_lanes(acc, x, l, l + 1, start);
+                start = (l + 1) * 16;
+                const uint32_t b2 = __float_as_uint(acc);
+                if (b2 == 0u || ts_fast(b2)) break;
+            }
+            scanned = false;
+            continue;
+        }
+        const int E = (int) ((bits >> 23) & 0xFF) - 127;
+        const uint32_t base = (bits & 0x7FFFFFu) | 0x800000u;
+        const float scale = __uint_as_float((uint32_t) (127 + 23 - E) << 23);
+        if (!scanned) { uint32_t total; ts_scan(x, start, scale, lane, s, fb, ex, total); off = 0; lane0 = 0; scanned = true; }
+        const uint32_t pre = base + ex - off;
+        const unsigned long long m = __ballot(lane >= lane0 && (fb < 16 || pre + s >= TS_TOP));
+        if (!m) {
+            const uint32_t total = (uint32_t) __shfl((int) (pre + s), 63);
+            return __uint_as_float(((uint32_t) (E + 127) << 23) | (total & 0x7FFFFFu));
+        }
+        const int L = __builtin_amdgcn_readfirstlane(__builtin_ctzll(m));
+        uint32_t run = pre; int r0 = 15;
+        bool open = true;
+#pragma unroll
+        for (int r = 0; r < 16; ++r) {
+            uint32_t q; (void) ts_units(x[r], scale, q);
+            if (lane * 16 + r >= start && open) { if (r == fb || run + q >= TS_TOP) { r0 = r; open = false; } else run += q; }
+        }
+        run = (uint32_t) __shfl((int) run, L);
+        r0 = __builtin_amdgcn_readfirstlane(__shfl(r0, L));
+        acc = ts_plain_lanes(__uint_as_float(((uint32_t) (E + 127) << 23) | (run & 0x7FFFFFu)), x, L, L + 1, L * 16 + r0);
+        start = (L + 1) * 16;
+        if (start >= 1024) break;
+        const uint32_t b2 = __float_as_uint(acc);
+        if (ts_fast(b2) && (int) ((b2 >> 23) & 0xFF) - 127 == E) { lane0 = L + 1; off = (uint32_t) __shfl((int) ex, L + 1); }
+        else scanned = false;
+    }
+    return acc;
+}
+
 __global__ __launch_bounds__(TS_W * 64) void k_ts_refine(const float * __restrict__ en_, const float * __restrict__ bmin_, const float * __restrict__ bmax_,
-                                                         int n_samples_, const TsTok * __restrict__ in, TsOut * __restrict__ out) {
-    __shared__ uint32_t s_sum[TS_W]; __shared__ int s_bad[TS_W]; __shared__ float s_acc;
+                                                         int n_samples_, const TsTok * __restrict__ in, TsOut * __restrict__ out,
+                                                         int * __restrict__ counter, int32_t * __restrict__ done, int32_t seq) {
+    __shared__ uint32_t s_sum[TS_W]; __shared__ float s_acc[2]; __shared__ int s_walk[4];
     const int tid = threadIdx.x, lane = tid & 63, wave = tid >> 6;
     const TsTok t = in[blockIdx.x];
     const float * __restrict__ en = t.en ? t.en : en_;
@@ -541,84 +641,117 @@
     const float * __restrict__ bmin = t.en ? t.en + t.ext_off : bmin_;
     const float * __restrict__ bmax = t.en ? bmin + ((size_t) t.n_samples / 256 + 2) : bmax_;
     float acc = 0.0f;
-    {
-        const float * p = en + t.a0;
-        const int n = t.a1 - t.a0;
-        auto fetch = [&](float (&dst)[16], int base) {
-#pragma unroll
-            for (int r = 0; r < 16; ++r) { const int e = base + r * 64 + lane; dst[r] = (e >= 0 && e < n) ? p[e] : 0.0f; }
+    if (t.a1 > t.a0) {
+        const long long a0 = t.a0, a1 = t.a1;
+        const long long g0 = a0 & ~3ll;
+        const int ntrips = (int) ((a1 - g0 + 1023) >> 10);
+        const bool aligned = ((uintptr_t) en & 15) == 0;
+        auto fetch = [&](float (&dst)[16], int trip) {
+            const long long g = g0 + (long long) trip * 1024 + lane * 16;
+#pragma unroll
+            for (int v = 0; v < 4; ++v) {
+                const long long gi = g + 4 * v;
+                if (aligned && gi >= a0 && gi + 4 <= a1) {
+                    const float4 f = *(const float4 *) (en + gi);
+                    dst[4 * v] = f.x; dst[4 * v + 1] = f.y; dst[4 * v + 2] = f.z; dst[4 * v + 3] = f.w;
+                } else {
+#pragma unroll
+                    for (int c = 0; c < 4; ++c) dst[4 * v + c] = (gi + c >= a0 && gi + c < a1) ? en[gi + c] : 0.0f;
+                }
+            }
         };
-        float x[16], nx[16]; int nx_base = -1;
-        int i = 0;
-        while (i < n) {
-            const int base = i + wave * 1024;
-            if (nx_base == base) {
-#pragma unroll
-                for (int r = 0; r < 16; ++r) x[r] = nx[r];
-            } else fetch(x, base);
-            nx_base = base + TS_W * 1024;
-            if (nx_base < n) fetch(nx, nx_base); else nx_base = -1;
+        float x[16], nx[16];
+#pragma unroll
+        for (int r = 0; r < 16; ++r) { x[r] = 0.0f; nx[r] = 0.0f; }
+        int tc = wave;
+        if (tc < ntrips) fetch(x, tc);
+        if (tc + TS_W < ntrips) fetch(nx, tc + TS_W);
+        auto advance = [&]() {
+#pragma unroll
+            for (int r = 0; r < 16; ++r) x[r] = nx[r];
+            tc += TS_W;
+            if (tc + TS_W < ntrips) fetch(nx, tc + TS_W);
+        };
+        if (wave == 0) {
+            const int nl = (int) ((a1 - g0 + 15) >> 4);
+            const float a2 = ts_plain_lanes(0.0f, x, 0, nl < 64 ? nl : 64, 0);
+            if (lane == 0) s_acc[1] = a2;
+            advance();
+        }
+        __syncthreads();
+        acc = s_acc[1];
+        int it = 0;
+        int T0 = 1;
+        while (T0 < ntrips) {
             const uint32_t bits = __float_as_uint(acc);
             const int E = (int) ((bits >> 23) & 0xFF) - 127;
-            const bool fast = (bits >> 31) == 0 && E >= -100 && E <= 100;
-            bool bad = !fast || base + 1024 > n;
-            uint32_t isum = 0;
-            if (!bad) {
-                const float scale = __uint_as_float((uint32_t) (127 + 23 - E) << 23);
-#pragma unroll
-                for (int r = 0; r < 16; ++r) {
-                    const float tt = x[r] * scale;
-                    const int q = __float2int_rn(tt);
-                    const float d = fabsf(tt - (float) q);
-                    bad = bad || d == 0.5f || !(tt < 8388608.0f) || tt < 0.0f;
-                    isum += (uint32_t) q;
+            const bool fast = ts_fast(bits);
+            uint32_t s = 0, ex = 0; int fb = 16;
+            if (tc < ntrips) {
+                uint32_t pub = TS_BAD;
+                if (bits == 0u) {
+                    bool nz = false;
+#pragma unroll
+                    for (int r = 0; r < 16; ++r) nz = nz || __float_as_uint(x[r]) != 0u;
+                    pub = __ballot(nz) ? TS_BAD : 0u;
+                } else if (fast) {
+                    uint32_t total;
+                    ts_scan(x, 0, __uint_as_float((uint32_t) (127 + 23 - E) << 23), lane, s, fb, ex, total);
+                    pub = __ballot(fb < 16) ? TS_BAD : total;
                 }
-                bad = bad || isum >= 0x1000000u;
-                bad = __ballot(bad) != 0;
-                if (!bad) { _Pragma("unroll") for (int o = 32; o > 0; o >>= 1) isum += (uint32_t) __shfl_xor((int) isum, o); }
-            }
-            if (lane == 0) { s_sum[wave] = isum; s_bad[wave] = bad ? 1 : 0; }
+                if (lane == 0) s_sum[wave] = pub;
+            }
             __syncthreads();
             int k = 0;
-            if (fast) {
-                uint32_t running = (bits & 0x7FFFFFu) | 0x800000u;
-                for (; k < TS_W; ++k) {
-                    if (s_bad[k] || (unsigned long long) running + s_sum[k] >= 0x1000000ull) break;
-                    running += s_sum[k];
+            for (;;) {
+                uint32_t run = fast ? ((__float_as_uint(acc) & 0x7FFFFFu) | 0x800000u) : 0u;
+                const int k0 = k;
+                for (; k < TS_W && T0 + k < ntrips; ++k) {
+                    const uint32_t v = s_sum[(T0 + k) & (TS_W - 1)];
+                    if (v == TS_BAD || run + v >= TS_TOP) break;
+                    run += v;
                 }
-                if (k > 0) acc = __uint_as_float(((uint32_t) (E + 127) << 23) | (running & 0x7FFFFFu));
-            }
-            i += k * 1024;
-            const bool slow = k < TS_W && i < n;
-            if (slow) {
-                if (wave == 0) {
-                    float y[16];
-                    if (k == 0) {
-#pragma unroll
-                        for (int r = 0; r < 16; ++r) y[r] = x[r];
-                    } else fetch(y, i);
-                    const float a2 = ts_trip_exact(acc, y, n - i, lane);
-                    if (lane == 0) s_acc = a2;
+                if (fast && k > k0) acc = __uint_as_float(((uint32_t) (E + 127) << 23) | (run & 0x7FFFFFu));
+                const int Ts = T0 + k;
+                if (!(k < TS_W && Ts < ntrips)) break;
+                if (tc == Ts) {
+                    const float a2 = ts_trip_onepass(acc, x, lane, fast, s, fb, ex);
+                    if (lane == 0) s_acc[it & 1] = a2;
                 }
                 __syncthreads();
-                acc = s_acc;
-                i += n - i < 1024 ? n - i : 1024;
-            }
+                acc = s_acc[it & 1];
+                ++it; ++k;
+                const uint32_t b2 = __float_as_uint(acc);
+                if (!(fast && ts_fast(b2) && (int) ((b2 >> 23) & 0xFF) - 127 == E)) break;
+            }
+            T0 += k;
+            if (tc < T0) advance();
             __syncthreads();
         }
     }
-    if (wave != 0) return;
     const int ns = t.a1 - t.a0;
     const float th = (float) (0.5 * (double) acc / (double) ns);
-    const float x0 = en[t.s0], x1 = en[t.s1];
-    const int wa = ts_walk(en, bmin, t.s0, 0, th, -1, true, lane);
-    const int wb = ts_walk(en, bmax, t.s0, t.s1, th, +1, false, lane);
-    const int wc = ts_walk(en, bmin, t.s1, n_samples - 1, th, +1, true, lane);
-    const int wd = ts_walk(en, bmax, t.s1, 0, th, -1, false, lane);
-    if (lane == 0) {
+    if (wave < 4) {
+        const int w = wave == 0 ? ts_walk(en, bmin, t.s0, 0, th, -1, true, lane)
+                    : wave == 1 ? ts_walk(en, bmax, t.s0, t.s1, th, +1, false, lane)
+                    : wave == 2 ? ts_walk(en, bmin, t.s1, n_samples - 1, th, +1, true, lane)
+                    :             ts_walk(en, bmax, t.s1, 0, th, -1, false, lane);
+        if (lane == 0) s_walk[wave] = w;
+    }
+    __syncthreads();
+    if (tid == 0) {
+        const float x0 = en[t.s0], x1 = en[t.s1];
         TsOut o; o.sum = acc; o.thold = th; o.e0 = x0 > th ? 1 : 0; o.e1 = x1 > th ? 1 : 0;
-        o.w_down_above_s0 = wa; o.w_up_below_s0 = wb; o.w_up_above_s1 = wc; o.w_down_below_s1 = wd;
+        o.w_down_above_s0 = s_walk[0]; o.w_up_below_s0 = s_walk[1]; o.w_up_above_s1 = s_walk[2]; o.w_down_below_s1 = s_walk[3];
         out[blockIdx.x] = o;
+        if (done) {
+            __threadfence_system();
+            if (atomicAdd(counter, 1) == (int) gridDim.x - 1) {
+                atomicExch(counter, 0);
+                __threadfence_system();
+                __hip_atomic_store(done, seq, __ATOMIC_RELEASE, __HIP_MEMORY_SCOPE_SYSTEM);
+            }
+        }
     }
 }
 constexpr int VB_ROW = VAD_BLOCK + 1;
@@ -740,8 +873,10 @@
     hipLaunchKernelGGL(k_vad_finish, dim3(1), dim3(128), 0, st, x, ys, n, n_last, alpha, nb, entry, exit_, vad_thold, res);
 }
 
-void ts_refine(const float * en, const float * bmin, const float * bmax, int n_samples, const TsTok * in, TsOut * out, int n_tok, hipStream_t st) {
-    if (n_tok > 0) hipLaunchKernelGGL(k_ts_refine, dim3(n_tok), dim3(TS_W * 64), 0, st, en, bmin, bmax, n_samples, in, out);
+void ts_refine(const float * en, const float * bmin, const float * bmax, int n_samples, const TsTok * in, TsOut * out, int n_tok, hipStream_t st,
+               int * counter, int32_t * done, int32_t seq) {
+    if (!counter) done = nullptr;
+    if (n_tok > 0) hipLaunchKernelGGL(k_ts_refine, dim3(n_tok), dim3(TS_W * 64), 0, st, en, bmin, bmax, n_samples, in, out, counter, done, seq);
 }
 
 void downmix_stereo(const float * frames, int n_frames, float * out, hipStream_t st) {
diff --git a/godot-whisper_amd/csrc/kernels.h b/godot-whisper_amd/csrc/kernels.h
--- a/godot-whisper_amd/csrc/kernels.h
+++ b/godot-whisper_amd/csrc/kernels.h
@@ -81,7 +81,8 @@
                const float * en; int32_t n_samples, ext_off; };
 struct TsOut { float sum, thold; int32_t e0, e1;
                int32_t w_down_above_s0, w_up_below_s0, w_up_above_s1, w_down_below_s1; };
-void ts_refine(const float * en, const float * bmin, const float * bmax, int n_samples, const TsTok * in, TsOut * out, int n_tok, hipStream_t st);
+void ts_refine(const float * en, const float * bmin, const float * bmax, int n_samples, const TsTok * in, TsOut * out, int n_tok, hipStream_t st,
+               int * counter = nullptr, int32_t * done = nullptr, int32_t seq = 0);
 
 void downmix_stereo(const float * frames, int n_frames, float * out, hipStream_t st);
 void vad_window(const float * x, int n, int n_last, float alpha, bool filter, float vad_thold, float * res, hipStream_t st);
diff --git a/godot-whisper_amd/csrc/wmi.h b/godot-whisper_amd/csrc/wmi.h
--- a/godot-whisper_amd/csrc/wmi.h
+++ b/godot-whisper_amd/csrc/wmi.h
@@ -178,6 +178,7 @@
     bool    energy_pending = false;
     bool    energy_device_only = false;
     void *  ts_host = nullptr;
+    int *   ts_count = nullptr; int32_t ts_seq = 0;
     __half * mel_t = nullptr;
     __half * conv1 = nullptr;
     float  * x     = nullptr;
@@ -473,6 +474,10 @@
 int busy_transcriptions(int device);
 bool signal_energy_device(whisper_context & ctx, int hw, bool sync = true, int via_dma = 0);
 bool ts_refine_device(State & st, const k::TsTok * in, int n, k::TsOut * out);
+bool ts_device_enabled();
+int  ts_poll_bound_us(int us);
+bool signal_energy_ready(State & st);
+hipStream_t envelope_stream_of(const State & st);
 struct TsRef { State * st; int seg, j; };
 bool flush_token_timestamps(whisper_context & ctx, State & st);
 bool flush_token_timestamps_of(whisper_context & ctx, const std::vector<State *> & states);
diff --git a/godot-whisper_amd/runtime.py b/godot-whisper_amd/runtime.py
--- a/godot-whisper_amd/runtime.py
+++ b/godot-whisper_amd/runtime.py
@@ -66,6 +66,7 @@
     ("wmi_downmix_stereo", C.c_int, [C.c_void_p, C.c_void_p, C.c_int, C.c_int, C.c_void_p]),
     ("wmi_vad", C.c_int, [C.c_void_p, C.c_void_p, C.c_int, C.c_int, C.c_float, C.c_float, C.c_void_p]),
     ("wmi_selftest_ts_refine", C.c_int, [C.c_void_p, C.c_void_p, C.c_int, C.c_void_p, C.c_int, C.c_void_p, C.c_void_p, C.c_void_p]),
+    ("wmi_selftest_ts_poll_us", C.c_int, [C.c_int]),
     ("wmi_selftest_resample_plan", C.c_int, [C.c_int, C.c_int, C.c_int, C.c_int, C.c_void_p, C.c_void_p, C.c_void_p, C.c_int, C.c_void_p,
                                              C.c_void_p]),
     ("wmi_resample", C.c_int, [C.c_void_p, C.c_void_p, C.c_int, C.c_int, C.c_int, C.c_int, C.c_int, C.c_void_p, C.c_int]),
diff --git a/include/wmi_device.h b/include/wmi_device.h
--- a/include/wmi_device.h
+++ b/include/wmi_device.h
@@ -109,6 +109,7 @@
 
 WHISPER_API int wmi_selftest_ts_refine(struct whisper_context * ctx, const float * envelope, int n, const int * s0s1, int n_tok,
                                        float * sums, float * thold, int * walks);
+WHISPER_API int wmi_selftest_ts_poll_us(int us);
 WHISPER_API int wmi_selftest_resample_plan(int n_frames, int src_rate, int dst_rate, int converter, long long * frames_gen,
                                            long long * frames_used, int * closed_form, int n_pos, long long * pos, double * frac);
 
diff --git a/scratch/lab/token_timestamps_cost.py b/scratch/lab/token_timestamps_cost.py
--- /dev/null
+++ b/scratch/lab/token_timestamps_cost.py
@@ -0,0 +1,57 @@
+import argparse
+import ctypes as C
+import json
+import pathlib
+import sys
+import time
+
+import numpy as np
+
+ap = argparse.ArgumentParser()
+ap.add_argument("--root", default=str(pathlib.Path(__file__).resolve().parents[2]))
+ap.add_argument("--reps", type=int, default=400)
+ap.add_argument("--warm", type=int, default=20)
+ap.add_argument("--shape", default="base.en")
+args = ap.parse_args()
+sys.path.insert(0, args.root)
+import __graft_entry__ as entry
+
+entry.load_package()
+from godot_whisper_amd import host, runtime, synth
+
+lib = runtime.require_gpu(); runtime.silence_logs(lib)
+node = host.SpeechToText(lib); node.set_language_model(synth.make_model(args.shape, seed=1234))
+pcms = [synth.make_pcm(30.0, seed=1234 + i) for i in range(8)]
+routes = {"token_timestamps": node.full_params("", 0), "without": node.full_params("", 0)}
+routes["without"].token_timestamps = False
+
+
+def call(p, i):
+    h = pcms[i % len(pcms)]
+    t0 = time.perf_counter()
+    ret = lib.whisper_full(node.ctx, p, h.ctypes.data_as(C.POINTER(C.c_float)), int(h.size))
+    dt = time.perf_counter() - t0
+    assert ret == 0, ret
+    return 1e3 * dt
+
+
+import gc
+times = {k: [] for k in routes}
+for i in range(args.warm + args.reps):
+    if i == args.warm:
+        gc.collect(); gc.freeze()
+    for name, p in routes.items():
+        dt = call(p, i)
+        if i >= args.warm:
+            times[name].append(dt)
+out = {"root": args.root, "shape": args.shape, "reps": args.reps}
+for name, v in times.items():
+    a = np.asarray(v)
+    out[name] = {"median_ms": round(float(np.median(a)), 4), "mean_ms": round(float(a.mean()), 4), "q25_ms": round(float(np.quantile(a, 0.25)), 4),
+                 "q75_ms": round(float(np.quantile(a, 0.75)), 4), "min_ms": round(float(a.min()), 4)}
+nblk = 10
+blk = [float(np.median(np.asarray(times["token_timestamps"])[b::nblk]) - np.median(np.asarray(times["without"])[b::nblk])) for b in range(nblk)]
+out["difference_of_medians_ms"] = round(out["token_timestamps"]["median_ms"] - out["without"]["median_ms"], 4)
+out["difference_over_ten_interleaved_subsets_ms"] = {"min": round(min(blk), 4), "max": round(max(blk), 4)}
+node.close()
+print("RESULT " + json.dumps(out))
```

Result: no change. 10830 x realtime (-0.3%).
